# ictnlp/StreamSpeech

Hardware: NVIDIA H100
Metric: audio-seconds/sec (RTF^-1) Fr-En simul S2ST @chunk=320ms (higher is better)
Workload: dtype f32

## Files before the change

### streamspeech_b200/csrc/engine.h

```cpp
#pragma once
#include <cuda_runtime.h>

#include <map>
#include <tuple>
#include <utility>
#include <string>
#include <vector>

#include "../../include/streamspeech_b200.h"
#include "kernels.h"
#include "kernels_persist.h"
#include "kernels_multistream.h"

namespace ss {

struct HostTensor {
  std::vector<float> data;
  std::vector<int64_t> shape;
  int64_t numel() const {
    int64_t n = 1;
    for (auto s : shape) n *= s;
    return n;
  }
};
// ... 12 lines not shown
struct ConformerLayerW {
  LNorm ffn1_ln, ffn2_ln, attn_ln, conv_ln, final_ln;
  Linear ffn1_w1, ffn1_w2, ffn2_w1, ffn2_w2;
  Linear qkv, attn_out;
  float* pos_u = nullptr;
  float* pos_v = nullptr;
  float* pos_proj = nullptr;
  Linear pw1;
  float* dw_w = nullptr;
  float* bn_scale = nullptr;
  float* bn_shift = nullptr;
  Linear pw2;
};

struct DecLayerW {
  LNorm self_ln, cross_ln, final_ln;
  Linear q, k, v, qkv, out;
  Linear cq, ckv, cout;
  Linear fc1, fc2;
  bool has_cross = false;
};

struct ConvW {
  Linear lin;
  int ksize = 1, cin = 0, cout = 0, dil = 1;
};

struct UpsampleW {
  int u = 1, k = 1, pad = 0, cin = 0, cout = 0;
  std::vector<Linear> phase_w;
  std::vector<int> phase_J, phase_q0;
  float* bias = nullptr;
};

struct Arena {
  char* base = nullptr;
  size_t cap = 0, off = 0;
  float* f32(size_t n) { return (float*)raw(n * 4); }
  void* raw(size_t bytes);
  void reset() { off = 0; }
  bool ensure(size_t bytes);
};

}

struct ss_engine {
  int device = 0;
  ss_config cfg{};
  std::string err;
  bool finalized = false;
  int attn_chunk = 8, conv_chunk = 8;
  int umma_vocoder = 0;
  int umma_linear = 0;
  int unit_grouped = 1;
  int umma_min_rows = 128;
  int umma_min_channels = 16;
  ss::Umma2Cache* umma2_cache = nullptr;
  int vocoder_streams = 1;
  cudaStream_t aux_stream[2] = {nullptr, nullptr};
  cudaEvent_t fork_event = nullptr, join_event[2] = {nullptr, nullptr};
  int vocoder_graph = 0;
  int graph_pdl = 0;
  cudaStream_t capture_stream = nullptr;
  std::map<std::tuple<int, uintptr_t, int, int, int>, std::pair<cudaGraphExec_t, int>> voc_graphs;
  int vocoder_fused = -1;
  std::map<std::pair<int, uintptr_t>, ss::VocFusedParams> voc_fused;
  float* persist_ffn_scratch = nullptr;
  float* cl_blobs = nullptr;
  int cluster_cooperative = 1;
  long long cl_steps = 0;
  int persistent_encoder_cluster = 0;
  int persistent_ffn_fused = 1;
  int fbank_tma = 1;
  int persistent_encoder = 1;
  std::map<std::string, ss::HostTensor> host;
  std::vector<void*> dev_allocs;

  ss::Linear sub_conv[2];
  ss::Linear enc_linear;
  std::vector<ss::ConformerLayerW> enc;
  int Tpos = 0;
  ss::Linear ctc_head[2];
  ss::Linear ctc_pair;
  unsigned* ctc_ticket = nullptr;
  float* mt_emb = nullptr;
  float* mt_pos = nullptr;
  int mt_pos_rows = 0;
  std::vector<ss::DecLayerW> mt;
  ss::LNorm mt_ln;
  std::vector<ss::DecLayerW> t2u;
  ss::LNorm t2u_ln;
  std::vector<ss::DecLayerW> unit;
  ss::LNorm unit_ln;
  float* unit_emb = nullptr;
  float* unit_pos_row = nullptr;
  float* mel_bank = nullptr;
  float* melT = nullptr;
  float* window = nullptr;
  float* cmvn_mean = nullptr;
  float* cmvn_std = nullptr;
  float* resample_h = nullptr;
  int resample_taps = 0, resample_width = 0;
  int* mask_pad_unk = nullptr;
  int* mask_pad_eos = nullptr;
  bool has_vocoder = false;
  float* voc_dict = nullptr;
  ss::ConvW dur_conv1, dur_conv2;
  ss::LNorm dur_ln1, dur_ln2;
  ss::Linear dur_proj;
  ss::ConvW conv_pre;
  std::vector<ss::UpsampleW> ups;
  std::vector<std::vector<std::vector<ss::ConvW>>> rb1, rb2;
  float* conv_post_w = nullptr;
  float conv_post_b = 0.f;
  int conv_post_k = 7, conv_post_c = 0;
  int hop = 1, receptive_field = 0;

  ss::Arena ws;
  float* mt_self_k = nullptr;
  float* mt_self_v = nullptr;
  float* mt_cross_kv = nullptr;
  int mt_cross_cap = 0;
  int mt_cross_final = 0;
  int mt_stable_hint = 0;
  const float* mt_cross_enc = nullptr;
  int mt_inc_self_len = 0;
  int mt_inc_cross_rows = 0;
  int64_t* mt_tok_dev = nullptr;
  int64_t* mt_next_dev = nullptr;
  int64_t* mt_next_pinned = nullptr;
  float* voc_unit_emb = nullptr;
  int* voc_cumsum = nullptr;
  int voc_ucap = 0, voc_U = 0;
  int st_T_final = 0;
  float* st_k = nullptr;
  float* st_v = nullptr;
  float* st_glu = nullptr;
  unsigned long long* persist_ts = nullptr;
  int persistent_profile = 0;
  int persistent_prefetch = 0;
  int persistent_time = 0;
  struct TimedLaunch { cudaEvent_t e0, e1; double bytes; };
  std::vector<TimedLaunch> time_events;
  std::vector<TimedLaunch> mt_time_events;
  ss::PersistLayer* persist_alias = nullptr;
  int persistent_alias = 0;
  unsigned* persist_bar = nullptr;
  unsigned persist_bar_target = 0;
  unsigned* async_err_pinned = nullptr;
  int persistent_barrier = 1;
  ss::MtLayerP* mt_persist_layers = nullptr;
  int persistent_mt = 1;
  int persistent_mt_v2 = 1;
  float* mt_part = nullptr;
  int persistent_mt_prefix = 1;
  ss::PersistLayer* persist_layers = nullptr;
  int* lengths_dev = nullptr;
  int lengths_cap = 0;

  struct StreamPool {
    int n_slots = 0, Tcap = 0, Fcap = 0;
    int64_t audio_cap = 0;
    float *audio = nullptr, *feats = nullptr, *k = nullptr, *v = nullptr, *glu = nullptr, *enc_out = nullptr, *melT = nullptr;
    int64_t* ctc_am = nullptr;
    ss::MsStream *desc_dev = nullptr, *desc_pinned = nullptr, *desc_dev2 = nullptr, *desc_pinned2 = nullptr;
    std::vector<int> T_final, n_feat;
    std::vector<int64_t> n_audio;
  } pool;

  int fail(int code, const std::string& msg) {
    err = msg;
    return code;
  }
};
```

### streamspeech_b200/csrc/engine_run.cu

```cuda
#include <algorithm>
#include <cmath>
#include <cstring>
#include <stdexcept>
#include <tuple>

#include "engine.h"

using namespace ss;

namespace {

inline cudaStream_t S(void* s) { return (cudaStream_t)s; }

int check_launch(ss_engine* h, const char* where) {
  cudaError_t e = cudaGetLastError();
  if (e != cudaSuccess) return h->fail(SS_ERR_CUDA, std::string(where) + ": " + cudaGetErrorString(e));
  return SS_OK;
}

thread_local int g_umma_linear = 0;
thread_local int g_umma_conv = 0;
thread_local int g_umma_min_rows = 128;
thread_local int g_umma_min_channels = 16;
thread_local Umma2Cache* g_umma2_cache = nullptr;
// ... 554 lines not shown
  if (T_final_out) *T_final_out = h->st_T_final;
  return check_launch(h, "ss_encoder_stream_step");
}

int ss_ctc_greedy_rows(ss_engine* h, void* stream, int head, const float* enc_dev, int rows, int row0, int64_t* argmax_dev,
                       int64_t* tokens_dev, int32_t* index_dev, int32_t* count_dev) {
  if (h) route_from(h);
  if (!h || !h->finalized) return h ? h->fail(SS_ERR_STATE, "engine not finalized") : SS_ERR_INVALID;
  if (head < 0 || head > 1 || rows <= 0 || row0 < 0 || row0 > rows) return h->fail(SS_ERR_INVALID, "bad ctc head / rows");
  const Linear& l = h->ctc_head[head];
  cudaStream_t st = S(stream);
  const int nr = rows - row0;
  if (nr > 0) {
    if (!ws_begin(h, (size_t)nr * l.N * sizeof(float) + 4096)) return h->fail(SS_ERR_CUDA, "workspace allocation failed");
    float* logits = h->ws.f32((size_t)nr * l.N);
    linear(enc_dev + (size_t)row0 * h->cfg.enc_dim, h->cfg.enc_dim, nr, l, ep_out(logits, l.N), st);
    argmax_rows(logits, l.N, nr, l.N, h->mask_pad_unk, 2, argmax_dev + row0, nullptr, st);
  }
  ctc_collapse(argmax_dev, rows, 0 , h->cfg.pad, tokens_dev, index_dev, count_dev, st);
  return check_launch(h, "ss_ctc_greedy");
}

int ss_ctc_greedy_pair(ss_engine* h, void* stream, const float* enc_dev, int rows, int row0, int64_t* argmax0_dev, int64_t* argmax1_dev,
                       int64_t* packed_out_dev) {
  if (h) route_from(h);
  if (!h || !h->finalized) return h ? h->fail(SS_ERR_STATE, "engine not finalized") : SS_ERR_INVALID;
  if (rows <= 0 || row0 < 0 || row0 > rows) return h->fail(SS_ERR_INVALID, "bad ctc rows");
  cudaStream_t st = S(stream);
  const int V = h->cfg.src_vocab;
  const int nr = rows - row0;
  const int W = 2 * rows + 2;
  if (h->ctc_pair.N != 2 * V || h->cfg.tgt_vocab != V) {
    for (int hd = 0; hd < 2; ++hd) {
      int64_t* o = packed_out_dev + (size_t)hd * W;
      int rc = ss_ctc_greedy_rows(h, stream, hd, enc_dev, rows, row0, hd ? argmax1_dev : argmax0_dev, o + 1, reinterpret_cast<int32_t*>(o + 1 + rows),
                                  reinterpret_cast<int32_t*>(o));
      if (rc) return rc;
    }
    return SS_OK;
  }
  float* logits = nullptr;
  if (nr > 0) {
    if (!ws_begin(h, (size_t)nr * 2 * V * sizeof(float) + 4096)) return h->fail(SS_ERR_CUDA, "workspace allocation failed");
    logits = h->ws.f32((size_t)nr * 2 * V);
    linear(enc_dev + (size_t)row0 * h->cfg.enc_dim, h->cfg.enc_dim, nr, h->ctc_pair, ep_out(logits, 2 * V), st);
  }
  ctc_argmax_collapse_pair(logits, 2 * V, V, nr, row0, rows, h->mask_pad_unk, 2, 0 , h->cfg.pad, argmax0_dev, argmax1_dev,
                           packed_out_dev, W, h->ctc_ticket, st);
  return check_launch(h, "ss_ctc_greedy_pair");
}

int ss_ctc_greedy(ss_engine* h, void* stream, int head, const float* enc_dev, int rows, int64_t* argmax_dev, int64_t* tokens_dev,
                  int32_t* index_dev, int32_t* count_dev) {
  return ss_ctc_greedy_rows(h, stream, head, enc_dev, rows, 0, argmax_dev, tokens_dev, index_dev, count_dev);
}

int ss_mt_features(ss_engine* h, void* stream, const float* enc_dev, int T, const int64_t* tokens_host, int n, float* feats_out_dev,
                   float* logits_last_dev) {
  if (h) route_from(h);
  if (!h || !h->finalized) return h ? h->fail(SS_ERR_STATE, "engine not finalized") : SS_ERR_INVALID;
  const ss_config& c = h->cfg;
  if (n <= 0 || n > c.max_mt_positions || T <= 0) return h->fail(SS_ERR_INVALID, "bad MT sequence length");
  cudaStream_t st = S(stream);
  int rc = ensure_mt_cross(h, T);
  if (rc) return rc;
  int n_valid = n;
  while (n_valid > 0 && tokens_host[n_valid - 1] == c.pad) --n_valid;
  for (int i = 0; i < n_valid; ++i)
    if (tokens_host[i] == c.pad) return h->fail(SS_ERR_INVALID, "pads are only supported as a tail");
  const int dim = c.mt_dim;
  if (!ws_begin(h, ((size_t)n * (dim * 7 + c.mt_ffn) + 4096) * sizeof(float))) return h->fail(SS_ERR_CUDA, "workspace allocation failed");
  DecScratch s = dec_scratch(h, n, dim, c.mt_ffn);
  float* x = h->ws.f32((size_t)n * dim);
  int* kvlen = nullptr;
  cudaMemcpyAsync(h->mt_tok_dev, tokens_host, n * sizeof(int64_t), cudaMemcpyHostToDevice, st);
  if (n_valid < n) {
    kvlen = (int*)h->ws.raw(sizeof(int));
    cudaMemcpyAsync(kvlen, &n_valid, sizeof(int), cudaMemcpyHostToDevice, st);
  }
  cudaStreamSynchronize(st);
  mt_begin(h, enc_dev, T, st);
  mt_forward(h, 0, n, T, kvlen, feats_out_dev, s, x, st);
  if (logits_last_dev) {
    Linear out;
    out.w = h->mt_emb; out.b = nullptr; out.N = c.tgt_vocab; out.K = dim;
    linear(feats_out_dev + (size_t)(n - 1) * dim, dim, 1, out, ep_out(logits_last_dev, c.tgt_vocab), st);
  }
  return check_launch(h, "ss_mt_features");
}

int ss_mt_greedy(ss_engine* h, void* stream, const float* enc_dev, int T, const int64_t* prefix_host, int n_prefix, int max_new_tokens,
                 int max_len_b, int64_t* tokens_out_host, int max_out, int* n_out, float* feats_out_dev) {
  if (h) route_from(h);
  if (!h || !h->finalized) return h ? h->fail(SS_ERR_STATE, "engine not finalized") : SS_ERR_INVALID;
  const ss_config& c = h->cfg;
  cudaStream_t st = S(stream);
  if (T <= 0 || n_prefix < 0 || !n_out) return h->fail(SS_ERR_INVALID, "bad arguments to ss_mt_greedy");
  const int start = n_prefix;
  int max_len = (max_new_tokens == -1) ? std::min(max_len_b, c.max_mt_positions - 1) : start + max_new_tokens;
  if (max_len < 1) return h->fail(SS_ERR_INVALID, "min_len cannot be larger than max_len");
  if (start > max_len) return h->fail(SS_ERR_INVALID, "prefix longer than max_len");
  if (max_len + 2 > c.max_mt_positions || max_len > max_out) return h->fail(SS_ERR_CAPACITY, "MT hypothesis longer than capacity");
  int rc = ensure_mt_cross(h, T);
  if (rc) return rc;
  const int dim = c.mt_dim;
  const int nmax = std::max(start + 1, 1);
  if (!ws_begin(h, ((size_t)nmax * (dim * 7 + c.mt_ffn) + c.tgt_vocab + 4096) * sizeof(float))) return h->fail(SS_ERR_CUDA, "workspace allocation failed");
  DecScratch s = dec_scratch(h, nmax, dim, c.mt_ffn);
  float* x = h->ws.f32((size_t)nmax * dim);
  float* logits = h->ws.f32(c.tgt_vocab);
  Linear outp;
  outp.w = h->mt_emb; outp.b = nullptr; outp.N = c.tgt_vocab; outp.K = dim;
  std::vector<int64_t> toks(start + 1);
  toks[0] = c.eos;
  for (int i = 0; i < start; ++i) toks[i + 1] = prefix_host[i];
  cudaMemcpyAsync(h->mt_tok_dev, toks.data(), toks.size() * sizeof(int64_t), cudaMemcpyHostToDevice, st);
  cudaStreamSynchronize(st);
  mt_begin(h, enc_dev, T, st);
  int fed = 0;
  int n_tok = start;
  for (int i = 0; i < start; ++i) tokens_out_host[i] = prefix_host[i];
  const int burst = (max_new_tokens >= 0) ? std::max(1, max_new_tokens) : 16;
  const bool persistent_mt = h->persistent_mt && mt_decode_persistent_supported(dim, c.mt_ffn, c.mt_heads, c.tgt_vocab, c.max_mt_positions, T);
  int step = start;
  bool done = false;
  if (persistent_mt && h->persistent_mt_prefix && h->persist_bar && start >= 1 && mt_prefix_persistent_supported(dim, c.mt_ffn, c.mt_heads, start, T)) {
    MtDecodeParams P;
    P.n_layers = c.mt_layers; P.heads = c.mt_heads; P.vocab = c.tgt_vocab; P.pad = c.pad; P.eos = c.eos;
    P.max_pos = c.max_mt_positions; P.cross_cap = h->mt_cross_cap;
    P.emb = h->mt_emb; P.pos = h->mt_pos; P.out_g = h->mt_ln.g; P.out_b = h->mt_ln.b;
    P.self_k = h->mt_self_k; P.self_v = h->mt_self_v; P.cross_kv = h->mt_cross_kv;
    P.tok = h->mt_tok_dev; P.feats = feats_out_dev; P.x = x; P.q = s.q; P.attn = s.attn; P.hid = s.hid; P.logits = logits;
        if (h->persistent_mt_v2 && h->mt_part) { P.part = h->mt_part; P.delta = h->mt_part + (size_t)8 * c.mt_dim; }
        if (h->persistent_profile) P.ts = h->persist_ts;
    if (mt_prefix_persistent(P, h->mt_persist_layers, start, T, h->persist_bar, &h->persist_bar_target, st) == 0)
      fed = start;
    else
      cudaGetLastError();
  }
  while (!done) {
    const int burst_first = step;
    int enq = 0;
    for (; step <= max_len && enq < burst; ++step, ++enq) {
      int n = step + 1 - fed;
      if (n == 1 && persistent_mt && h->persist_bar) {
        const int cnt = std::min(max_len - step + 1, burst - enq);
        MtDecodeParams P;
        P.n_layers = c.mt_layers; P.heads = c.mt_heads; P.vocab = c.tgt_vocab; P.pad = c.pad; P.eos = c.eos;
        P.max_pos = c.max_mt_positions; P.cross_cap = h->mt_cross_cap;
        P.emb = h->mt_emb; P.pos = h->mt_pos; P.out_g = h->mt_ln.g; P.out_b = h->mt_ln.b;
        P.self_k = h->mt_self_k; P.self_v = h->mt_self_v; P.cross_kv = h->mt_cross_kv;
        P.tok = h->mt_tok_dev; P.feats = feats_out_dev; P.x = x; P.q = s.q; P.attn = s.attn; P.hid = s.hid; P.logits = logits;
        if (h->persistent_mt_v2 && h->mt_part) { P.part = h->mt_part; P.delta = h->mt_part + (size_t)8 * c.mt_dim; }
        if (h->persistent_profile) P.ts = h->persist_ts;
        cudaEvent_t ev0 = nullptr, ev1 = nullptr;
        if (h->persistent_time && h->mt_time_events.size() < 4096 && cudaEventCreate(&ev0) == cudaSuccess && cudaEventCreate(&ev1) == cudaSuccess)
          cudaEventRecord(ev0, st);
        else
          ev0 = ev1 = nullptr;
        const int rc_launch = mt_decode_persistent(P, h->mt_persist_layers, step, cnt, max_len, T, h->persist_bar, &h->persist_bar_target, st);
        if (ev0 && ev1) {
          cudaEventRecord(ev1, st);
          h->mt_time_events.push_back({ev0, ev1, -1.0});
        }
        if (rc_launch == 0) {
          fed = step + cnt;
          if (step + cnt - 1 >= max_len) done = true;
          step += cnt;
          enq += cnt;
          break;
        }
        cudaGetLastError();
      }
      mt_forward(h, fed, n, T, nullptr, feats_out_dev + (size_t)fed * dim, s, x, st);
      fed = step + 1;
      if (step >= max_len) {
        done = true;
        ++step;
        break;
      }
      linear(feats_out_dev + (size_t)step * dim, dim, 1, outp, ep_out(logits, c.tgt_vocab), st);
      if (step < 1)
        argmax_rows(logits, c.tgt_vocab, 1, c.tgt_vocab, h->mask_pad_eos, 2, h->mt_tok_dev + step + 1, nullptr, st);
      else
        argmax_rows(logits, c.tgt_vocab, 1, c.tgt_vocab, h->mask_pad_unk, 1, h->mt_tok_dev + step + 1, nullptr, st);
    }
    int produced = step - burst_first - (done ? 1 : 0);
    if (produced > 0) {
      cudaMemcpyAsync(h->mt_next_pinned, h->mt_tok_dev + burst_first + 1, produced * sizeof(int64_t), cudaMemcpyDeviceToHost, st);
      if (h->persist_bar && h->async_err_pinned)
        cudaMemcpyAsync(h->async_err_pinned, h->persist_bar + SS_BAR_ERR_WORD, sizeof(unsigned), cudaMemcpyDeviceToHost, st);
      if (cudaStreamSynchronize(st) != cudaSuccess)
        return h->fail(SS_ERR_CUDA, std::string("ss_mt_greedy: ") + cudaGetErrorString(cudaGetLastError()));
      if (h->async_err_pinned && *h->async_err_pinned) {
        const unsigned f = *h->async_err_pinned;
        *h->async_err_pinned = 0;
        return report_async_error(h, f, "ss_mt_greedy");
      }
      int steps_run = produced;
      for (int i = 0; i < produced; ++i) {
        int64_t next = h->mt_next_pinned[i];
        if (next == c.eos) {
          done = true;
          steps_run = i + 1;
          break;
        }
        tokens_out_host[n_tok++] = next;
      }
      if (!h->mt_time_events.empty() && h->mt_time_events.back().bytes < 0.0) h->mt_time_events.back().bytes = (double)steps_run;
    }
    if (step > max_len) done = true;
  }
  *n_out = n_tok;
  return check_launch(h, "ss_mt_greedy");
}

int ss_mt_incremental_reset(ss_engine* h) {
  if (!h) return SS_ERR_INVALID;
  h->mt_inc_self_len = 0;
  h->mt_inc_cross_rows = 0;
  return SS_OK;
}

int ss_mt_greedy_incremental(ss_engine* h, void* stream, const float* enc_dev, int T, const int64_t* prefix_host, int n_prefix,
                             int max_new_tokens, int max_len_b, int64_t* tokens_out_host, int max_out, int* n_out) {
  if (h) route_from(h);
  if (!h || !h->finalized) return h ? h->fail(SS_ERR_STATE, "engine not finalized") : SS_ERR_INVALID;
  const ss_config& c = h->cfg;
  cudaStream_t st = S(stream);
  if (T <= 0 || n_prefix < 0 || !n_out) return h->fail(SS_ERR_INVALID, "bad arguments to ss_mt_greedy_incremental");
  const int start = n_prefix;
  const int max_len = (max_new_tokens == -1) ? max_len_b : start + max_new_tokens;
  if (max_len < 1) return h->fail(SS_ERR_INVALID, "min_len cannot be larger than max_len");
  if (start > max_len) return h->fail(SS_ERR_INVALID, "prefix longer than max_len");
  const int kv_off = h->mt_inc_self_len - start;
  if (kv_off < 0) return h->fail(SS_ERR_STATE, "incremental MT state is shorter than the prefix (reset missing, or a prefix that this state did not produce)");
  if (max_len + kv_off + 2 > c.max_mt_positions || max_len > max_out) return h->fail(SS_ERR_CAPACITY, "MT hypothesis longer than capacity");
  if (!h->persistent_mt || !h->persist_bar || !mt_decode_persistent_supported(c.mt_dim, c.mt_ffn, c.mt_heads, c.tgt_vocab, c.max_mt_positions, std::max(T, h->mt_inc_cross_rows)))
    return h->fail(SS_ERR_STATE, "incremental MT decoding runs on the persistent MT kernel, which is off or does not support this shape");
  int rc = ensure_mt_cross(h, std::max(T, h->mt_inc_cross_rows), h->mt_inc_cross_rows);
  if (rc) return rc;
  const int dim = c.mt_dim;
  if (!ws_begin(h, ((size_t)(dim * 8 + c.mt_ffn) + c.tgt_vocab + (size_t)c.max_mt_positions * dim + 4096) * sizeof(float))) return h->fail(SS_ERR_CUDA, "workspace allocation failed");
  DecScratch s = dec_scratch(h, 1, dim, c.mt_ffn);
  float* x = h->ws.f32(dim);
  float* logits = h->ws.f32(c.tgt_vocab);
  float* feats = h->ws.f32((size_t)c.max_mt_positions * dim);
  if (!x || !logits || !feats) return h->fail(SS_ERR_CUDA, "workspace too small");
  if (h->mt_inc_cross_rows == 0) {
    h->mt_cross_final = 0;
    h->mt_cross_enc = nullptr;
  }
  if (T > h->mt_inc_cross_rows) {
    const int from = h->mt_inc_cross_rows;
    for (int l = 0; l < c.mt_layers; ++l) {
      float* cross = h->mt_cross_kv + (size_t)l * h->mt_cross_cap * 2 * dim;
      linear(enc_dev + (size_t)from * c.enc_dim, c.enc_dim, T - from, h->mt[l].ckv, ep_out(cross + (size_t)from * 2 * dim, 2 * dim), st);
    }
    h->mt_inc_cross_rows = T;
  }
  const int Tk = h->mt_inc_cross_rows;
  std::vector<int64_t> toks(start + 1);
  toks[0] = c.eos;
  for (int i = 0; i < start; ++i) toks[i + 1] = prefix_host[i];
  cudaMemcpyAsync(h->mt_tok_dev, toks.data(), toks.size() * sizeof(int64_t), cudaMemcpyHostToDevice, st);
  cudaStreamSynchronize(st);
  int n_tok = start;
  for (int i = 0; i < start; ++i) tokens_out_host[i] = prefix_host[i];
  const int burst = (max_new_tokens >= 0) ? std::max(1, max_new_tokens + 1) : 32;
  int step = start;
  bool done = false;
  while (!done) {
    const int cnt = std::min(max_len - step + 1, burst);
    MtDecodeParams P;
    P.n_layers = c.mt_layers; P.heads = c.mt_heads; P.vocab = c.tgt_vocab; P.pad = c.pad; P.eos = c.eos;
    P.max_pos = c.max_mt_positions; P.cross_cap = h->mt_cross_cap; P.kv_off = kv_off;
    P.emb = h->mt_emb; P.pos = h->mt_pos; P.out_g = h->mt_ln.g; P.out_b = h->mt_ln.b;
    P.self_k = h->mt_self_k; P.self_v = h->mt_self_v; P.cross_kv = h->mt_cross_kv;
    P.tok = h->mt_tok_dev; P.feats = feats; P.x = x; P.q = s.q; P.attn = s.attn; P.hid = s.hid; P.logits = logits;
        if (h->persistent_mt_v2 && h->mt_part) { P.part = h->mt_part; P.delta = h->mt_part + (size_t)8 * c.mt_dim; }
        if (h->persistent_profile) P.ts = h->persist_ts;
    if (mt_decode_persistent(P, h->mt_persist_layers, step, cnt, max_len, Tk, h->persist_bar, &h->persist_bar_target, st) != 0) {
      cudaGetLastError();
      return h->fail(SS_ERR_CUDA, "cooperative launch of the persistent MT kernel was refused");
    }
    const int readable = std::min(cnt, max_len - step);
    if (readable > 0) cudaMemcpyAsync(h->mt_next_pinned, h->mt_tok_dev + step + 1, readable * sizeof(int64_t), cudaMemcpyDeviceToHost, st);
    if (h->async_err_pinned) cudaMemcpyAsync(h->async_err_pinned, h->persist_bar + SS_BAR_ERR_WORD, sizeof(unsigned), cudaMemcpyDeviceToHost, st);
    if (cudaStreamSynchronize(st) != cudaSuccess) return h->fail(SS_ERR_CUDA, std::string("ss_mt_greedy_incremental: ") + cudaGetErrorString(cudaGetLastError()));
    if (h->async_err_pinned && *h->async_err_pinned) {
      const unsigned f = *h->async_err_pinned;
      *h->async_err_pinned = 0;
      return report_async_error(h, f, "ss_mt_greedy_incremental");
    }
    for (int i = 0; i < cnt && !done; ++i) {
      const int sidx = step + i;
      h->mt_inc_self_len = sidx + kv_off + 1;
      if (sidx >= max_len) { done = true; break; }
      const int64_t next = h->mt_next_pinned[i];
      if (next == c.eos) { done = true; break; }
      tokens_out_host[n_tok++] = next;
    }
    step += cnt;
    if (step > max_len) done = true;
  }
  *n_out = n_tok;
  return check_launch(h, "ss_mt_greedy_incremental");
}

int ss_t2u_unit_decode(ss_engine* h, void* stream, const float* mt_feats_dev, int Slen, int n_pad_tail, int mask_eos, int64_t* argmax_dev,
                       int64_t* units_dev, int32_t* count_dev, float* t2u_out_dev, float* logits_dev) {
  if (h) route_from(h);
  if (!h || !h->finalized) return h ? h->fail(SS_ERR_STATE, "engine not finalized") : SS_ERR_INVALID;
  const ss_config& c = h->cfg;
  cudaStream_t st = S(stream);
  if (Slen <= 0 || n_pad_tail < 0 || n_pad_tail >= Slen) return h->fail(SS_ERR_INVALID, "bad T2U sequence length");
  const int dim = c.unit_dim, R = c.ctc_upsample_rate, L = Slen * R;
  size_t need = ((size_t)L * (dim * 8 + c.unit_ffn + c.unit_vocab) + (size_t)Slen * dim * 12 + (size_t)Slen * c.unit_ffn + 8192) * sizeof(float);
  if (!ws_begin(h, need)) return h->fail(SS_ERR_CUDA, "workspace allocation failed");
  DecScratch s1 = dec_scratch(h, Slen, dim, c.unit_ffn);
  float* x = h->ws.f32((size_t)Slen * dim);
  float* t2u = t2u_out_dev ? t2u_out_dev : h->ws.f32((size_t)Slen * dim);
  int* kvlen = nullptr;
  int* kvlen_up = nullptr;
  if (n_pad_tail > 0) {
    int v[2] = {Slen - n_pad_tail, (Slen - n_pad_tail) * R};
    kvlen = (int*)h->ws.raw(2 * sizeof(int));
    kvlen_up = kvlen + 1;
    cudaMemcpyAsync(kvlen, v, sizeof(v), cudaMemcpyHostToDevice, st);
    cudaStreamSynchronize(st);
  }
  copy_f32(mt_feats_dev, x, (int64_t)Slen * dim, st);
  for (int l = 0; l < c.t2u_layers; ++l)
    dec_layer(h->t2u[l], x, Slen, dim, c.unit_ffn, c.unit_heads, c.uni_encoder != 0, 0, kvlen, nullptr, nullptr, 0, nullptr, 0, nullptr, s1, st);
  layer_norm(x, dim, t2u, dim, h->t2u_ln.g, h->t2u_ln.b, Slen, dim, st);
  DecScratch s2 = dec_scratch(h, L, dim, c.unit_ffn);
  float* xu = h->ws.f32((size_t)L * dim);
  float* ckv = h->ws.f32((size_t)Slen * 2 * dim);
  float* logits = logits_dev ? logits_dev : h->ws.f32((size_t)L * c.unit_vocab);
  if (!xu || !ckv || !logits) return h->fail(SS_ERR_CUDA, "workspace too small");
  repeat_rows_add(t2u, Slen, R, dim, h->unit_pos_row, xu, st);
  for (int l = 0; l < c.unit_layers; ++l) {
    linear(t2u, dim, Slen, h->unit[l].ckv, ep_out(ckv, 2 * dim), st);
    const int gR = (l == 0 && h->unit_grouped) ? R : 0;
    dec_layer(h->unit[l], xu, L, dim, c.unit_ffn, c.unit_heads, true, 0, kvlen_up, nullptr, nullptr, 0, ckv, Slen, kvlen, s2, st, gR, kvlen);
  }
  layer_norm(xu, dim, xu, dim, h->unit_ln.g, h->unit_ln.b, L, dim, st);
  Linear outp;
  outp.w = h->unit_emb; outp.b = nullptr; outp.N = c.unit_vocab; outp.K = dim;
  linear(xu, dim, L, outp, ep_out(logits, c.unit_vocab), st);
  argmax_rows(logits, c.unit_vocab, L, c.unit_vocab, h->mask_pad_unk, mask_eos ? 3 : 2, argmax_dev, nullptr, st);
  ctc_collapse(argmax_dev, L, c.unit_vocab - 1, c.pad, units_dev, nullptr, count_dev, st);
  return check_launch(h, "ss_t2u_unit_decode");
}

int ss_unit_position_row(ss_engine* h, const float* row_host) {
  if (!h || !h->finalized || !row_host) return h ? h->fail(SS_ERR_STATE, "engine not finalized / null row") : SS_ERR_INVALID;
  cudaDeviceSynchronize();
  if (cudaMemcpy(h->unit_pos_row, row_host, (size_t)h->cfg.unit_dim * sizeof(float), cudaMemcpyHostToDevice) != cudaSuccess)
    return h->fail(SS_ERR_CUDA, "cudaMemcpy(unit positional row) failed");
  return SS_OK;
}

int ss_vocoder_durations(ss_engine* h, void* stream, const int64_t* codes_dev, int U, int dur_prediction, int64_t* dur_out_dev,
                         int32_t* cumsum_out_dev) {
  if (!h || !h->finalized) return h ? h->fail(SS_ERR_STATE, "engine not finalized") : SS_ERR_INVALID;
  if (!h->has_vocoder) return h->fail(SS_ERR_STATE, "no vocoder weights were loaded");
  if (U <= 0) return h->fail(SS_ERR_INVALID, "empty code sequence");
  const ss_config& c = h->cfg;
  cudaStream_t st = S(stream);
  const int E = c.voc_embedding_dim, Hd = c.voc_dur_hidden;
  if (U > h->voc_ucap) {
    if (h->voc_unit_emb) cudaFree(h->voc_unit_emb);
    if (h->voc_cumsum) cudaFree(h->voc_cumsum);
    h->voc_unit_emb = nullptr;
    h->voc_cumsum = nullptr;
    h->voc_ucap = 0;
    const int cap = std::max(2 * U, 1024);
    if (cudaMalloc((void**)&h->voc_unit_emb, (size_t)cap * E * sizeof(float)) != cudaSuccess ||
        cudaMalloc((void**)&h->voc_cumsum, (size_t)(cap + 1) * sizeof(int)) != cudaSuccess)
      return h->fail(SS_ERR_CUDA, "cudaMalloc(vocoder unit cache) failed");
    h->voc_ucap = cap;
  }
  h->voc_U = U;
  if (!ws_begin(h, ((size_t)U * (2 * Hd + 2) + 4096) * sizeof(float))) return h->fail(SS_ERR_CUDA, "workspace allocation failed");
  gather_rows(codes_dev, U, 0, h->voc_dict, E, h->voc_unit_emb, st);
  float* a = h->ws.f32((size_t)U * Hd);
  float* b = h->ws.f32((size_t)U * Hd);
  float* ld = h->ws.f32(U);
  if (dur_prediction) {
    ConvA c1;
    c1.x = h->voc_unit_emb; c1.B = 1; c1.L_in = U; c1.L_rows = U; c1.C_in = E; c1.ldx = E;
    c1.ksize = h->dur_conv1.ksize; c1.pad_left = (h->dur_conv1.ksize - 1) / 2;
    Epilogue e1 = ep_out(a, Hd, ACT_RELU);
    e1.bias = h->dur_conv1.lin.b;
    gemm_conv(c1, h->dur_conv1.lin.w, Hd, e1, st);
    layer_norm(a, Hd, a, Hd, h->dur_ln1.g, h->dur_ln1.b, U, Hd, st);
    ConvA c2;
    c2.x = a; c2.B = 1; c2.L_in = U; c2.L_rows = U; c2.C_in = Hd; c2.ldx = Hd;
    c2.ksize = h->dur_conv2.ksize; c2.pad_left = 1;
    Epilogue e2 = ep_out(b, Hd, ACT_RELU);
    e2.bias = h->dur_conv2.lin.b;
    gemm_conv(c2, h->dur_conv2.lin.w, Hd, e2, st);
    layer_norm(b, Hd, b, Hd, h->dur_ln2.g, h->dur_ln2.b, U, Hd, st);
    linear(b, Hd, U, h->dur_proj, ep_out(ld, 1), st);
  } else {
    std::vector<float> v(U, 0.6931472f);
    cudaMemcpyAsync(ld, v.data(), U * sizeof(float), cudaMemcpyHostToDevice, st);
    cudaStreamSynchronize(st);
  }
  duration_from_log(ld, U, dur_out_dev, h->voc_cumsum, st);
  if (cumsum_out_dev) cudaMemcpyAsync(cumsum_out_dev, h->voc_cumsum, (U + 1) * sizeof(int), cudaMemcpyDeviceToDevice, st);
  return check_launch(h, "ss_vocoder_durations");
}

int ss_vocoder_generate(ss_engine* h, void* stream, int total_frames, int frame0, int n_frames, int left_context, float* wav_out_dev) {
  if (!h || !h->finalized) return h ? h->fail(SS_ERR_STATE, "engine not finalized") : SS_ERR_INVALID;
  if (!h->has_vocoder || h->voc_U <= 0) return h->fail(SS_ERR_STATE, "ss_vocoder_durations must run first");
  if (n_frames <= 0 || frame0 < 0 || frame0 + n_frames != total_frames) return h->fail(SS_ERR_INVALID, "vocoder frame range must be the tail of the sequence");
  const ss_config& c = h->cfg;
  cudaStream_t st = S(stream);
  route_from(h);
  g_umma_conv = h->umma_vocoder;
  int ctx = left_context < 0 ? h->receptive_field : left_context;
  ctx = std::min(ctx, frame0);
  const int f_lo = frame0 - ctx;
  const int N = n_frames + ctx;
  size_t maxbuf = 0;
  {
    int ch = c.voc_init_channels;
    size_t L = N;
    maxbuf = L * ch;
    for (int i = 0; i < c.voc_n_ups; ++i) {
// ... 68 lines not shown
      a.pre_lrelu = 0.1f;
      Epilogue e = ep_out(bufY, U.cout);
      e.bias = U.bias;
      e.out_L = Lout; e.out_row_stride = U.u; e.out_row_offset = q0 * U.u + phi - U.pad;
      conv_gemm(a, U.phase_w[phi].w, U.cout, e, sp);
    }
    set_splitk_slot(0);
    if (fan_up)
      for (int q = 0; q < 2; ++q) {
        cudaEventRecord(h->join_event[q], h->aux_stream[q]);
        cudaStreamWaitEvent(st, h->join_event[q], 0);
      }
    L = Lout;
    ch = U.cout;
    if (fan_out) {
      cudaEventRecord(h->fork_event, st);
      for (int q = 0; q < 2; ++q) cudaStreamWaitEvent(h->aux_stream[q], h->fork_event, 0);
    }
    for (int j = 0; j < nrb; ++j) {
      cudaStream_t sj = (fan_out && j > 0) ? h->aux_stream[j - 1] : st;
      set_splitk_slot(fan_out ? j : 0);
      const float* cur = bufY;
      float* pingpong[2] = {rbA[j], rbB[j]};
      int nd = c.voc_rb_ndil;
      for (int m = 0; m < nd; ++m) {
        const ConvW& w1 = h->rb1[i][j][m];
        const ConvW& w2 = h->rb2[i][j][m];
        ConvA a1;
        a1.x = cur; a1.B = 1; a1.L_in = L; a1.L_rows = L; a1.C_in = ch; a1.ldx = ch; a1.ksize = w1.ksize; a1.dil = w1.dil;
        a1.pad_left = (w1.ksize * w1.dil - w1.dil) / 2; a1.pre_lrelu = 0.1f;
        Epilogue e1 = ep_out(rbT[j], ch);
        e1.bias = w1.lin.b;
        conv_gemm(a1, w1.lin.w, ch, e1, sj);
        ConvA a2;
        a2.x = rbT[j]; a2.B = 1; a2.L_in = L; a2.L_rows = L; a2.C_in = ch; a2.ldx = ch; a2.ksize = w2.ksize; a2.dil = 1;
        a2.pad_left = (w2.ksize - 1) / 2; a2.pre_lrelu = 0.1f;
        Epilogue e2;
        e2.bias = w2.lin.b;
        e2.ldo = ch;
        e2.residual = cur;
        if (m + 1 < nd) {
          e2.out = pingpong[m & 1];
          e2.res_scale = 1.0f;
        } else {
          e2.out = nrb == 3 ? rbO[j] : bufX;
          e2.alpha = 1.0f / nrb;
          e2.res_scale = 1.0f / nrb;
          e2.accumulate = nrb != 3 && j > 0;
        }
        conv_gemm(a2, w2.lin.w, ch, e2, sj);
        cur = e2.out;
      }
      if (fan_out && j > 0) cudaEventRecord(h->join_event[j - 1], sj);
    }
    set_splitk_slot(0);
    if (fan_out)
      for (int q = 0; q < 2; ++q) cudaStreamWaitEvent(st, h->join_event[q], 0);
    if (nrb == 3) add3_f32(rbO[0], rbO[1], rbO[2], bufX, (int64_t)L * ch, st);
  }
  conv_post_tanh(bufX, L, ch, h->conv_post_w, h->conv_post_b, h->conv_post_k, 0.01f, wav, st);
  };
  bool replayed = false;
  if (h->vocoder_graph) {
    const auto key = std::make_tuple(N, (uintptr_t)h->ws.base, g_umma_conv, g_umma_min_rows * 4096 + g_umma_min_channels, h->vocoder_streams);
    auto it = h->voc_graphs.find(key);
    if (it != h->voc_graphs.end()) {
      if (cudaGraphLaunch(it->second.first, st) == cudaSuccess) {
        g_launches += it->second.second;
        replayed = true;
      } else {
        cudaGetLastError();
      }
    } else {
      generator_body(st);
      replayed = true;
      if (!h->capture_stream) cudaStreamCreateWithFlags(&h->capture_stream, cudaStreamNonBlocking);
      const unsigned long long before = g_launches;
      if (h->capture_stream && cudaStreamBeginCapture(h->capture_stream, cudaStreamCaptureModeRelaxed) == cudaSuccess) {
        g_pdl_off = h->graph_pdl ? 0 : 1;
        generator_body(h->capture_stream);
        g_pdl_off = 0;
        cudaGraph_t graph = nullptr;
        cudaGraphExec_t exec = nullptr;
        if (cudaStreamEndCapture(h->capture_stream, &graph) == cudaSuccess && graph != nullptr &&
            cudaGraphInstantiate(&exec, graph, 0) == cudaSuccess) {
          h->voc_graphs[key] = std::make_pair(exec, (int)(g_launches - before));
        } else {
          cudaGetLastError();
          h->vocoder_graph = 0;
        }
        if (graph) cudaGraphDestroy(graph);
      } else {
        cudaGetLastError();
        h->vocoder_graph = 0;
      }
      g_launches = before;
    }
  }
  if (!replayed) generator_body(st);
  copy_f32(wav + (size_t)ctx * h->hop, wav_out_dev, (int64_t)n_frames * h->hop, st);
  return check_launch(h, "ss_vocoder_generate");
}

int ss_set_option(ss_engine* h, const char* name, int value) {
  if (!h || !name) return SS_ERR_INVALID;
  std::string n(name);
  if (n == "umma_vocoder") h->umma_vocoder = value;
  else if (n == "umma_linear") h->umma_linear = value;
  else if (n == "umma_min_rows") h->umma_min_rows = value;
  else if (n == "umma_min_channels") h->umma_min_channels = value;
  else if (n == "umma2_cache_clear") {
    umma2_cache_clear(h->umma2_cache);
    clear_graphs(h);
  }
  else if (n == "umma2_split_below") { g_umma2_split_below = value; clear_graphs(h); }
  else if (n == "umma2_min_units") { g_umma2_min_units = value; clear_graphs(h); }
  else if (n == "umma2_debug") {
    if (value && !g_umma2_dbg) {
      if (cudaMalloc(&g_umma2_dbg, 16 * sizeof(unsigned long long)) != cudaSuccess) return h->fail(SS_ERR_CUDA, "cudaMalloc failed");
      cudaMemset(g_umma2_dbg, 0, 16 * sizeof(unsigned long long));
    }
    if (!value && g_umma2_dbg) {
      cudaDeviceSynchronize();
      cudaFree(g_umma2_dbg);
      g_umma2_dbg = nullptr;
    }
  }
  else if (n == "prefer_shared") g_prefer_shared = value;
  else if (n == "unit_grouped") h->unit_grouped = value;
  else if (n == "vocoder_graph") h->vocoder_graph = value;
  else if (n == "vocoder_fused") h->vocoder_fused = value;
  else if (n == "graph_pdl") h->graph_pdl = value;
  else if (n == "fbank_tma") h->fbank_tma = value;
  else if (n == "umma2_fused_reduce") g_umma2_fused_reduce = value;
  else if (n == "persistent_encoder") h->persistent_encoder = value;
  else if (n == "persistent_ffn_fused") h->persistent_ffn_fused = value;
  else if (n == "cluster_cooperative") h->cluster_cooperative = value;
  else if (n == "persistent_encoder_cluster") {
    if (value && !h->cl_blobs) {
      if (!h->persist_layers || !h->persist_bar) return h->fail(SS_ERR_STATE, "persistent_encoder_cluster needs a finalized engine");
      const size_t n_f = encoder_layers_cluster_blob_floats(h->cfg.enc_layers);
      if (h->cfg.enc_dim != 256 || h->cfg.enc_ffn != 2048) return h->fail(SS_ERR_INVALID, "persistent_encoder_cluster: encoder must be 256 / 2048");
      if (cudaMalloc(&h->cl_blobs, n_f * sizeof(float)) != cudaSuccess) return h->fail(SS_ERR_CUDA, "cudaMalloc failed");
      h->dev_allocs.push_back(h->cl_blobs);
      encoder_layers_cluster_pack(h->persist_layers, h->cfg.enc_layers, h->cfg.dw_kernel, h->cl_blobs, 0);
      if (cudaDeviceSynchronize() != cudaSuccess) return h->fail(SS_ERR_CUDA, "packing the cluster weight blobs failed");
    }
    h->persistent_encoder_cluster = value;
  }
  else if (n == "vocoder_streams") h->vocoder_streams = value;
  else if (n == "persistent_mt") h->persistent_mt = value;
  else if (n == "persistent_mt_prefix") h->persistent_mt_prefix = value;
  else if (n == "persistent_mt_v2") h->persistent_mt_v2 = value;
  else if (n == "persistent_prefetch") h->persistent_prefetch = value;
  else if (n == "persistent_time") h->persistent_time = value;
  else if (n == "persistent_barrier") {
    if (value && !h->persist_bar) {
      if (cudaMalloc(&h->persist_bar, 256) != cudaSuccess) return h->fail(SS_ERR_CUDA, "cudaMalloc failed");
      h->dev_allocs.push_back(h->persist_bar);
      cudaMemset(h->persist_bar, 0, 256);
      h->persist_bar_target = 0;
    }
    h->persistent_barrier = value;
  }
  else if (n == "persistent_alias") {
    if (value && !h->persist_alias) {
      const int L = h->cfg.enc_layers;
      if (cudaMalloc(&h->persist_alias, L * sizeof(PersistLayer)) != cudaSuccess) return h->fail(SS_ERR_CUDA, "cudaMalloc failed");
      h->dev_allocs.push_back(h->persist_alias);
      for (int i = 0; i < L; ++i) cudaMemcpy(h->persist_alias + i, h->persist_layers, sizeof(PersistLayer), cudaMemcpyDeviceToDevice);
    }
    h->persistent_alias = value;
  }
  else if (n == "persistent_profile") {
    if (value && !h->persist_ts) {
      if (cudaMalloc(&h->persist_ts, 4096 * sizeof(unsigned long long)) != cudaSuccess) return h->fail(SS_ERR_CUDA, "cudaMalloc failed");
      h->dev_allocs.push_back(h->persist_ts);
    }
    h->persistent_profile = value;
  }
  else return h->fail(SS_ERR_INVALID, "unknown option " + n);
  return SS_OK;
}

int ss_debug_copy(ss_engine* h, const char* what, void* host_dst, size_t bytes) {
  if (!h || !what || !host_dst) return SS_ERR_INVALID;
  std::string n(what);
  if (n == "persist_ts") {
    if (!h->persist_ts || bytes > 4096 * sizeof(unsigned long long)) return h->fail(SS_ERR_STATE, "no phase timestamps (set option persistent_profile)");
    if (cudaMemcpy(host_dst, h->persist_ts, bytes, cudaMemcpyDeviceToHost) != cudaSuccess) return h->fail(SS_ERR_CUDA, "cudaMemcpy failed");
    return SS_OK;
  }
  if (n == "umma2_ts") {
    if (!g_umma2_dbg || bytes > 16 * sizeof(unsigned long long)) return h->fail(SS_ERR_STATE, "no stamps (set option umma2_debug)");
    if (cudaMemcpy(host_dst, g_umma2_dbg, bytes, cudaMemcpyDeviceToHost) != cudaSuccess) return h->fail(SS_ERR_CUDA, "cudaMemcpy failed");
    return SS_OK;
  }
  if (n == "cluster_steps") {
    if (bytes < sizeof(long long)) return h->fail(SS_ERR_INVALID, "cluster_steps needs a long long");
    *(long long*)host_dst = h->cl_steps;
    return SS_OK;
  }
  if (n == "mt_time") {
    if (bytes < 3 * sizeof(double)) return h->fail(SS_ERR_INVALID, "mt_time needs 3 doubles");
    cudaDeviceSynchronize();
    double* out = (double*)host_dst;
    out[0] = out[1] = out[2] = 0.0;
    for (auto& e : h->mt_time_events) {
      float ms = 0.f;
      if (e.bytes >= 0.0 && cudaEventElapsedTime(&ms, e.e0, e.e1) == cudaSuccess) {
        out[0] += ms;
        out[1] += 1.0;
        out[2] += e.bytes;
      }
      cudaEventDestroy(e.e0);
      cudaEventDestroy(e.e1);
    }
    cudaGetLastError();
    h->mt_time_events.clear();
    return SS_OK;
  }
  if (n == "persist_time") {
    if (bytes < 3 * sizeof(double)) return h->fail(SS_ERR_INVALID, "persist_time needs 3 doubles");
    cudaDeviceSynchronize();
    double* out = (double*)host_dst;
    out[0] = out[1] = out[2] = 0.0;
    for (auto& e : h->time_events) {
      float ms = 0.f;
      if (cudaEventElapsedTime(&ms, e.e0, e.e1) == cudaSuccess) {
        out[0] += ms;
        out[1] += 1.0;
        out[2] += e.bytes;
      }
      cudaEventDestroy(e.e0);
      cudaEventDestroy(e.e1);
    }
    cudaGetLastError();
    h->time_events.clear();
    return SS_OK;
  }
  return h->fail(SS_ERR_INVALID, "unknown debug buffer " + n);
}

int ss_op_linear_umma(ss_engine* h, void* stream, const float* x_dev, int M, int K, const float* w_dev, const float* bias_dev, int N, int act,
                      int pieces, float* out_dev) {
  if (!h) return SS_ERR_INVALID;
  route_from(h);
  if (pieces != 2 && pieces != 3) return h->fail(SS_ERR_INVALID, "pieces must be 2 (bf16x3) or 3 (bf16x6)");
  ConvA a;
  a.x = x_dev; a.B = 1; a.L_in = M; a.L_rows = M; a.C_in = K; a.ldx = K;
  Epilogue ep = ep_out(out_dev, N, act);
  ep.bias = bias_dev;
  if (!umma2_supported(a, N, ep)) return h->fail(SS_ERR_INVALID, "shape not supported by the wgmma kernel");
  umma2_conv(h->umma2_cache, a, w_dev, N, ep, pieces, S(stream));
  return check_launch(h, "ss_op_linear_umma");
}

int ss_op_conv1d(ss_engine* h, void* stream, const float* x_dev, int L, int C_in, const float* w_dev, const float* bias_dev, int N, int ksize,
                 int dil, int pad_left, float pre_lrelu, int mode, float* out_dev) {
  if (!h) return SS_ERR_INVALID;
  route_from(h);
  ConvA a;
  a.x = x_dev; a.B = 1; a.L_in = L; a.L_rows = L; a.C_in = C_in; a.ldx = C_in; a.ksize = ksize; a.dil = dil; a.pad_left = pad_left;
  a.pre_lrelu = pre_lrelu;
  Epilogue ep = ep_out(out_dev, N);
  ep.bias = bias_dev;
  if (mode >= 12) {
    if (!umma2_supported(a, N, ep)) return h->fail(SS_ERR_INVALID, "shape not supported by the wgmma conv kernel");
    umma2_conv(h->umma2_cache, a, w_dev, N, ep, mode - 10, S(stream));
  } else if (mode >= 2) {
    return h->fail(SS_ERR_INVALID, "modes 2 / 3 (first-generation tensor-core kernel) were removed: use 12 / 13");
  } else {
    gemm_conv(a, w_dev, N, ep, S(stream));
  }
  return check_launch(h, "ss_op_conv1d");
}

int ss_op_linear(ss_engine* h, void* stream, const float* x_dev, int M, int K, const float* w_dev, const float* bias_dev, int N, int act,
                 float* out_dev) {
  if (!h) return SS_ERR_INVALID;
  Linear l;
  l.w = const_cast<float*>(w_dev); l.b = const_cast<float*>(bias_dev); l.N = N; l.K = K;
  linear(x_dev, K, M, l, ep_out(out_dev, N, act), S(stream));
  return check_launch(h, "ss_op_linear");
}

int ss_op_layer_norm(ss_engine* h, void* stream, const float* x_dev, int rows, int C, const float* g_dev, const float* b_dev, float* out_dev) {
  if (!h) return SS_ERR_INVALID;
  layer_norm(x_dev, C, out_dev, C, g_dev, b_dev, rows, C, S(stream));
  return check_launch(h, "ss_op_layer_norm");
}

}

#include "engine_pool.inc"
```

### streamspeech_b200/csrc/engine_weights.cu

```cuda
#include <cstdio>
#include <cstring>
#include <cmath>
#include <stdexcept>

#include "engine.h"

using namespace ss;

namespace ss {

void* Arena::raw(size_t bytes) {
  size_t a = (off + 255) & ~(size_t)255;
  if (a + bytes > cap) return nullptr;
  off = a + bytes;
  return base + a;
}

bool Arena::ensure(size_t bytes) {
  if (bytes <= cap) return true;
  if (base) cudaFree(base);
  base = nullptr;
  cap = 0;
  size_t want = bytes + (bytes >> 2) + (1 << 20);
  if (cudaMalloc((void**)&base, want) != cudaSuccess) return false;
// ... 146 lines not shown
    {
      std::vector<float> t((size_t)257 * 80);
      for (int m = 0; m < 80; ++m)
        for (int k = 0; k < 257; ++k) t[(size_t)k * 80 + m] = mb.data[(size_t)m * 257 + k];
      h->melT = upload(h, t);
    }
    const HostTensor& w = get(h, "__const__.window");
    expect_shape(w, "__const__.window", {400});
    h->window = upload(h, w.data);
    if (h->host.count("__const__.gcmvn_mean")) {
      h->cmvn_mean = upload(h, get(h, "__const__.gcmvn_mean").data);
      h->cmvn_std = upload(h, get(h, "__const__.gcmvn_std").data);
    }
    if (h->host.count("__const__.resample_3to1")) {
      const HostTensor& r = get(h, "__const__.resample_3to1");
      if (r.numel() < 4 || r.numel() > 64 || (r.numel() - 3) % 2 != 0) throw std::runtime_error("bad __const__.resample_3to1");
      h->resample_h = upload(h, r.data);
      h->resample_taps = (int)r.numel();
      h->resample_width = ((int)r.numel() - 3) / 2;
    }
    int m[3] = {c.pad, c.unk, c.eos};
    h->mask_pad_unk = dev_alloc<int>(h, 3);
    cudaMemcpy(h->mask_pad_unk, m, sizeof(m), cudaMemcpyHostToDevice);
    int m2[2] = {c.pad, c.eos};
    h->mask_pad_eos = dev_alloc<int>(h, 2);
    cudaMemcpy(h->mask_pad_eos, m2, sizeof(m2), cudaMemcpyHostToDevice);
  }
  {
    ConvW c0 = make_conv(h, "encoder.subsample.conv_layers.0", c.conv_channels, c.feat_dim, c.conv_kernel, 1, true);
    ConvW c1 = make_conv(h, "encoder.subsample.conv_layers.1", 2 * D, c.conv_channels / 2, c.conv_kernel, 1, true);
    h->sub_conv[0] = c0.lin;
    h->sub_conv[1] = c1.lin;
    h->enc_linear = make_linear(h, "encoder.linear", D, D);
  }
  const HostTensor& pe = get(h, "__const__.enc_pe");
  h->Tpos = c.max_enc_frames;
  expect_shape(pe, "__const__.enc_pe", {2 * (int64_t)h->Tpos - 1, D});
  std::vector<float> pe_flipped(pe.data.size());
  const int P = 2 * h->Tpos - 1;
  for (int k = 0; k < P; ++k) memcpy(&pe_flipped[(size_t)(P - 1 - k) * D], &pe.data[(size_t)k * D], D * sizeof(float));
  float* pe_dev = upload(h, pe_flipped);
  h->enc.resize(c.enc_layers);
  for (int i = 0; i < c.enc_layers; ++i) {
    ConformerLayerW& L = h->enc[i];
    std::string p = "encoder.conformer_layers." + std::to_string(i);
    L.ffn1_ln = make_ln(h, p + ".ffn1.layer_norm", D);
    L.ffn1_w1 = make_linear(h, p + ".ffn1.w_1", c.enc_ffn, D);
    L.ffn1_w2 = make_linear(h, p + ".ffn1.w_2", D, c.enc_ffn);
    L.ffn2_ln = make_ln(h, p + ".ffn2.layer_norm", D);
    L.ffn2_w1 = make_linear(h, p + ".ffn2.w_1", c.enc_ffn, D);
    L.ffn2_w2 = make_linear(h, p + ".ffn2.w_2", D, c.enc_ffn);
    L.attn_ln = make_ln(h, p + ".self_attn_layer_norm", D);
    L.qkv = make_fused(h, {p + ".self_attn.linear_q", p + ".self_attn.linear_k", p + ".self_attn.linear_v"}, D, D);
    L.attn_out = make_linear(h, p + ".self_attn.linear_out", D, D);
    L.pos_u = upload(h, get(h, p + ".self_attn.pos_bias_u").data);
    L.pos_v = upload(h, get(h, p + ".self_attn.pos_bias_v").data);
    Linear lp = make_linear(h, p + ".self_attn.linear_pos", D, D, false);
    L.pos_proj = dev_alloc<float>(h, (size_t)P * D);
    ConvA a;
    a.x = pe_dev; a.B = 1; a.L_in = P; a.L_rows = P; a.C_in = D; a.ldx = D;
    Epilogue ep;
    ep.out = L.pos_proj; ep.ldo = D;
    gemm_conv(a, lp.w, D, ep, 0);
    L.conv_ln = make_ln(h, p + ".conv_module.layer_norm", D);
    ConvW pw1 = make_conv(h, p + ".conv_module.pointwise_conv1", 2 * D, D, 1, 1, true, false);
    L.pw1 = pw1.lin;
    {
      const HostTensor& dw = get(h, p + ".conv_module.depthwise_conv.weight");
      expect_shape(dw, p + ".conv_module.depthwise_conv.weight", {D, 1, c.dw_kernel});
      std::vector<float> t((size_t)c.dw_kernel * D);
      for (int ch = 0; ch < D; ++ch)
        for (int k = 0; k < c.dw_kernel; ++k) t[(size_t)k * D + ch] = dw.data[(size_t)ch * c.dw_kernel + k];
      L.dw_w = upload(h, t);
      const auto& g = get(h, p + ".conv_module.batch_norm.weight").data;
      const auto& b = get(h, p + ".conv_module.batch_norm.bias").data;
      const auto& rm = get(h, p + ".conv_module.batch_norm.running_mean").data;
      const auto& rv = get(h, p + ".conv_module.batch_norm.running_var").data;
      std::vector<float> sc(D), sh(D);
      for (int ch = 0; ch < D; ++ch) {
        float inv = 1.0f / std::sqrt(rv[ch] + 1e-5f);
        sc[ch] = g[ch] * inv;
        sh[ch] = b[ch] - rm[ch] * g[ch] * inv;
      }
      L.bn_scale = upload(h, sc);
      L.bn_shift = upload(h, sh);
    }
    ConvW pw2 = make_conv(h, p + ".conv_module.pointwise_conv2", D, D, 1, 1, false, false);
    L.pw2 = pw2.lin;
    L.final_ln = make_ln(h, p + ".final_layer_norm", D);
  }
  {
    size_t n = (size_t)c.enc_layers * h->Tpos * D;
    h->st_k = dev_alloc<float>(h, n);
    h->st_v = dev_alloc<float>(h, n);
    h->st_glu = dev_alloc<float>(h, n);
    std::vector<PersistLayer> pl(c.enc_layers);
    for (int i = 0; i < c.enc_layers; ++i) {
      const ConformerLayerW& L = h->enc[i];
      PersistLayer& q = pl[i];
      q.ffn1_g = L.ffn1_ln.g; q.ffn1_b = L.ffn1_ln.b; q.ffn1_w1 = L.ffn1_w1.w; q.ffn1_b1 = L.ffn1_w1.b; q.ffn1_w2 = L.ffn1_w2.w; q.ffn1_b2 = L.ffn1_w2.b;
      q.attn_g = L.attn_ln.g; q.attn_b = L.attn_ln.b; q.wqkv = L.qkv.w; q.bqkv = L.qkv.b; q.wo = L.attn_out.w; q.bo = L.attn_out.b;
      q.pos_u = L.pos_u; q.pos_v = L.pos_v; q.pos_proj = L.pos_proj;
      q.conv_g = L.conv_ln.g; q.conv_b = L.conv_ln.b; q.pw1 = L.pw1.w; q.pw1_b = L.pw1.b; q.dw_w = L.dw_w; q.bn_scale = L.bn_scale;
      q.bn_shift = L.bn_shift; q.pw2 = L.pw2.w; q.pw2_b = L.pw2.b;
      q.ffn2_g = L.ffn2_ln.g; q.ffn2_b = L.ffn2_ln.b; q.ffn2_w1 = L.ffn2_w1.w; q.ffn2_b1 = L.ffn2_w1.b; q.ffn2_w2 = L.ffn2_w2.w; q.ffn2_b2 = L.ffn2_w2.b;
      q.fin_g = L.final_ln.g; q.fin_b = L.final_ln.b;
      for (int which = 0; which < 2; ++which) {
        const HostTensor& w2 = get(h, "encoder.conformer_layers." + std::to_string(&q - pl.data()) + (which ? ".ffn2.w_2.weight" : ".ffn1.w_2.weight"));
        std::vector<float> t((size_t)c.enc_ffn * D);
        for (int n = 0; n < D; ++n)
          for (int u = 0; u < c.enc_ffn; ++u) t[(size_t)u * D + n] = w2.data[(size_t)n * c.enc_ffn + u];
        (which ? q.ffn2_w2t : q.ffn1_w2t) = upload(h, t);
      }
    }
    h->persist_ffn_scratch = dev_alloc<float>(h, (size_t)(c.enc_ffn / 16) * 16 * D);
    h->persist_layers = dev_alloc<PersistLayer>(h, pl.size());
    cudaMemcpy(h->persist_layers, pl.data(), pl.size() * sizeof(PersistLayer), cudaMemcpyHostToDevice);
    h->persist_bar = dev_alloc<unsigned>(h, 64);
    cudaMemset(h->persist_bar, 0, 64 * sizeof(unsigned));
    h->persist_bar_target = 0;
    if (!h->async_err_pinned && cudaHostAlloc((void**)&h->async_err_pinned, sizeof(unsigned), cudaHostAllocDefault) == cudaSuccess)
      *h->async_err_pinned = 0;
  }
  if (c.src_vocab == c.tgt_vocab) {
    h->ctc_pair = make_fused(h, {"source_unigram_decoder.proj", "ctc_target_unigram_decoder.proj"}, c.src_vocab, D);
    h->ctc_head[0] = h->ctc_pair;
    h->ctc_head[0].N = c.src_vocab;
    h->ctc_head[1] = h->ctc_pair;
    h->ctc_head[1].N = c.tgt_vocab;
    h->ctc_head[1].w = h->ctc_pair.w + (size_t)c.src_vocab * D;
    h->ctc_head[1].b = h->ctc_pair.b + c.src_vocab;
  } else {
    h->ctc_head[0] = make_linear(h, "source_unigram_decoder.proj", c.src_vocab, D);
    h->ctc_head[1] = make_linear(h, "ctc_target_unigram_decoder.proj", c.tgt_vocab, D);
  }
  h->ctc_ticket = dev_alloc<unsigned>(h, 8);
  cudaMemset(h->ctc_ticket, 0, 8 * sizeof(unsigned));
  {
    const HostTensor& e = get(h, "target_unigram_decoder.embed_tokens.weight");
    expect_shape(e, "target_unigram_decoder.embed_tokens.weight", {c.tgt_vocab, c.mt_dim});
    h->mt_emb = upload(h, e.data);
    const HostTensor& pt = get(h, "__const__.mt_pos_table");
    if (pt.shape.size() != 2 || pt.shape[1] != c.mt_dim) throw std::runtime_error("bad __const__.mt_pos_table");
    h->mt_pos_rows = (int)pt.shape[0];
    h->mt_pos = upload(h, pt.data);
    for (int i = 0; i < c.mt_layers; ++i)
      h->mt.push_back(make_dec_layer(h, "target_unigram_decoder.layers." + std::to_string(i), c.mt_dim, c.mt_ffn, D, true));
    h->mt_ln = make_ln(h, "target_unigram_decoder.layer_norm", c.mt_dim);
    size_t cache = (size_t)c.mt_layers * c.max_mt_positions * c.mt_dim;
    h->mt_self_k = dev_alloc<float>(h, cache);
    h->mt_self_v = dev_alloc<float>(h, cache);
    h->mt_tok_dev = dev_alloc<int64_t>(h, c.max_mt_positions + 8);
    h->mt_next_dev = dev_alloc<int64_t>(h, 8);
    h->mt_part = dev_alloc<float>(h, (size_t)9 * c.mt_dim);
    cudaMallocHost((void**)&h->mt_next_pinned, (size_t)(c.max_mt_positions + 8) * sizeof(int64_t));
    std::vector<MtLayerP> ml(c.mt_layers);
    for (int i = 0; i < c.mt_layers; ++i) {
      const DecLayerW& L = h->mt[i];
      MtLayerP& q = ml[i];
      q.self_g = L.self_ln.g; q.self_b = L.self_ln.b; q.wqkv = L.qkv.w; q.bqkv = L.qkv.b; q.wo = L.out.w; q.bo = L.out.b;
      q.cross_g = L.cross_ln.g; q.cross_b = L.cross_ln.b; q.wcq = L.cq.w; q.bcq = L.cq.b; q.wco = L.cout.w; q.bco = L.cout.b;
      q.fin_g = L.final_ln.g; q.fin_b = L.final_ln.b; q.w1 = L.fc1.w; q.b1 = L.fc1.b; q.w2 = L.fc2.w; q.b2 = L.fc2.b;
    }
    h->mt_persist_layers = dev_alloc<MtLayerP>(h, ml.size());
    cudaMemcpy(h->mt_persist_layers, ml.data(), ml.size() * sizeof(MtLayerP), cudaMemcpyHostToDevice);
  }
  for (int i = 0; i < c.t2u_layers; ++i)
    h->t2u.push_back(make_dec_layer(h, "synthesizer_encoder.layers." + std::to_string(i), c.unit_dim, c.unit_ffn, c.unit_dim, false));
  h->t2u_ln = make_ln(h, "synthesizer_encoder.layer_norm", c.unit_dim);
  for (int i = 0; i < c.unit_layers; ++i)
    h->unit.push_back(make_dec_layer(h, "decoder.layers." + std::to_string(i), c.unit_dim, c.unit_ffn, c.unit_dim, true));
  h->unit_ln = make_ln(h, "decoder.layer_norm", c.unit_dim);
  {
    const HostTensor& e = get(h, "decoder.embed_tokens.weight");
    expect_shape(e, "decoder.embed_tokens.weight", {c.unit_vocab, c.unit_dim});
    h->unit_emb = upload(h, e.data);
    const HostTensor& pr = get(h, "__const__.unit_pos_row");
    expect_shape(pr, "__const__.unit_pos_row", {c.unit_dim});
    h->unit_pos_row = upload(h, pr.data);
  }
  h->has_vocoder = h->host.count("vocoder.dict.weight") > 0;
  if (h->has_vocoder) {
    const int E = c.voc_embedding_dim;
    const HostTensor& dict = get(h, "vocoder.dict.weight");
    expect_shape(dict, "vocoder.dict.weight", {c.voc_num_embeddings, E});
    h->voc_dict = upload(h, dict.data);
    h->dur_conv1 = make_conv(h, "vocoder.dur_predictor.conv1.0", c.voc_dur_hidden, E, c.voc_dur_kernel, 1, false);
    h->dur_ln1 = make_ln(h, "vocoder.dur_predictor.ln1", c.voc_dur_hidden);
    h->dur_conv2 = make_conv(h, "vocoder.dur_predictor.conv2.0", c.voc_dur_hidden, c.voc_dur_hidden, c.voc_dur_kernel, 1, false);
    h->dur_ln2 = make_ln(h, "vocoder.dur_predictor.ln2", c.voc_dur_hidden);
    h->dur_proj = make_linear(h, "vocoder.dur_predictor.proj", 1, c.voc_dur_hidden);
    h->conv_pre = make_conv(h, "vocoder.conv_pre", c.voc_init_channels, c.voc_in_dim, 7, 1, false);
    int ch = c.voc_init_channels;
    h->hop = 1;
    h->rb1.resize(c.voc_n_ups);
    h->rb2.resize(c.voc_n_ups);
    for (int i = 0; i < c.voc_n_ups; ++i) {
      UpsampleW U;
      U.u = c.voc_up_rates[i];
      U.k = c.voc_up_kernels[i];
      U.pad = (U.k - U.u) / 2;
      U.cin = ch;
      U.cout = ch / 2;
      if ((U.k - U.u) % 2 != 0 || U.pad >= U.u + U.k) throw std::runtime_error("unsupported upsample geometry");
      h->hop *= U.u;
      const std::string p = "vocoder.ups." + std::to_string(i);
      const HostTensor& w = get(h, p + ".weight");
      expect_shape(w, p + ".weight", {U.cin, U.cout, U.k});
      U.bias = upload(h, get(h, p + ".bias").data);
      for (int phi = 0; phi < U.u; ++phi) {
        int J = (U.k - phi + U.u - 1) / U.u;
        std::vector<float> pw((size_t)U.cout * J * U.cin);
        for (int co = 0; co < U.cout; ++co)
          for (int jp = 0; jp < J; ++jp) {
            int kk = phi + (J - 1 - jp) * U.u;
            for (int ci = 0; ci < U.cin; ++ci)
              pw[((size_t)co * J + jp) * U.cin + ci] = w.data[((size_t)ci * U.cout + co) * U.k + kk];
          }
        Linear l;
        l.N = U.cout;
        l.K = J * U.cin;
        l.w = upload(h, pw);
        l.b = U.bias;
        U.phase_w.push_back(l);
        U.phase_J.push_back(J);
        U.phase_q0.push_back(phi < U.pad ? (U.pad - phi + U.u - 1) / U.u : 0);
      }
      h->ups.push_back(U);
      ch = U.cout;
      h->rb1[i].resize(c.voc_n_rb);
      h->rb2[i].resize(c.voc_n_rb);
      for (int j = 0; j < c.voc_n_rb; ++j) {
        int rb = i * c.voc_n_rb + j;
        int rk = c.voc_rb_kernels[j];
        for (int m = 0; m < c.voc_rb_ndil; ++m) {
          std::string q = "vocoder.resblocks." + std::to_string(rb);
          h->rb1[i][j].push_back(make_conv(h, q + ".convs1." + std::to_string(m), ch, ch, rk, c.voc_rb_dils[j][m], false));
          h->rb2[i][j].push_back(make_conv(h, q + ".convs2." + std::to_string(m), ch, ch, rk, 1, false));
        }
      }
    }
    {
      const HostTensor& w = get(h, "vocoder.conv_post.weight");
      expect_shape(w, "vocoder.conv_post.weight", {1, ch, 7});
      std::vector<float> t((size_t)7 * ch);
      for (int ci = 0; ci < ch; ++ci)
        for (int k = 0; k < 7; ++k) t[(size_t)k * ch + ci] = w.data[(size_t)ci * 7 + k];
      h->conv_post_w = upload(h, t);
      h->conv_post_b = get(h, "vocoder.conv_post.bias").data[0];
      h->conv_post_c = ch;
      h->conv_post_k = 7;
    }
    int maxk = 0, sumd = 0;
    for (int j = 0; j < c.voc_n_rb; ++j) {
      int s = 0;
      for (int m = 0; m < c.voc_rb_ndil; ++m) s += c.voc_rb_dils[j][m] + 1;
      int r = (c.voc_rb_kernels[j] - 1) / 2 * s;
      if (r > maxk) maxk = r;
      (void)sumd;
    }
    int r = 3;
    for (int i = c.voc_n_ups - 1; i >= 0; --i) {
      r += maxk;
      r = (r + c.voc_up_kernels[i] + c.voc_up_rates[i] - 1) / c.voc_up_rates[i] + 1;
    }
    h->receptive_field = r + 3;
  }
  if (cudaDeviceSynchronize() != cudaSuccess) throw std::runtime_error(std::string("CUDA error during finalize: ") + cudaGetErrorString(cudaGetLastError()));
  h->host.clear();
  h->finalized = true;
}

}

extern "C" {

const char* ss_version(void) { return "streamspeech_b200 0.1 (sm_90a)"; }

int ss_create(ss_engine** out, int device, const ss_config* cfg) {
  if (!out || !cfg) return SS_ERR_INVALID;
  *out = nullptr;
  int n = 0;
  if (cudaGetDeviceCount(&n) != cudaSuccess || n <= 0 || device >= n) return SS_ERR_CUDA;
  if (cudaSetDevice(device) != cudaSuccess) return SS_ERR_CUDA;
  ss_engine* h = new ss_engine();
  h->device = device;
  h->cfg = *cfg;
  if (h->cfg.voc_n_ups > SS_MAX_UPS || h->cfg.voc_n_rb > SS_MAX_RB || h->cfg.voc_rb_ndil > SS_MAX_DIL) {
    delete h;
    return SS_ERR_INVALID;
  }
  *out = h;
  return SS_OK;
}

int ss_destroy(ss_engine* h) {
  if (!h) return SS_OK;
  cudaSetDevice(h->device);
  cudaDeviceSynchronize();
  for (void* p : h->dev_allocs) cudaFree(p);
  for (auto& kv : h->voc_graphs) cudaGraphExecDestroy(kv.second.first);
  h->voc_graphs.clear();
  if (h->capture_stream) cudaStreamDestroy(h->capture_stream);
  ss::umma2_cache_destroy(h->umma2_cache);
  if (h->ws.base) cudaFree(h->ws.base);
  if (h->mt_cross_kv) cudaFree(h->mt_cross_kv);
  if (h->mt_next_pinned) cudaFreeHost(h->mt_next_pinned);
// ... 58 lines not shown
```

### streamspeech_b200/csrc/kernels_persist.h

```cpp
#pragma once
#include <cuda_runtime.h>
#include <stdint.h>

namespace ss {

#define SS_BAR_ERR_WORD 32

#ifdef __CUDACC__
__device__ __forceinline__ void grid_barrier(unsigned* ctr, unsigned& target) {
  __syncthreads();
  target += gridDim.x;
  if (threadIdx.x == 0) {
    asm volatile("red.release.gpu.global.add.u32 [%0], 1;" ::"l"(ctr) : "memory");
    unsigned v, spins = 0;
    do {
      asm volatile("ld.relaxed.gpu.global.u32 %0, [%1];" : "=r"(v) : "l"(ctr) : "memory");
    } while ((int)(v - target) < 0 && ++spins < (1u << 20));
    if ((int)(v - target) < 0) atomicExch(ctr + SS_BAR_ERR_WORD, 1u);
    asm volatile("fence.acq_rel.gpu;" ::: "memory");
  }
  __syncthreads();
}
#endif

struct PersistLayer {
  const float *ffn1_g, *ffn1_b, *ffn1_w1, *ffn1_b1, *ffn1_w2, *ffn1_b2;
  const float *attn_g, *attn_b, *wqkv, *bqkv, *wo, *bo, *pos_u, *pos_v, *pos_proj;
  const float *conv_g, *conv_b, *pw1, *pw1_b, *dw_w, *bn_scale, *bn_shift, *pw2, *pw2_b;
  const float *ffn2_g, *ffn2_b, *ffn2_w1, *ffn2_b1, *ffn2_w2, *ffn2_b2;
  const float *fin_g, *fin_b;
  const float *ffn1_w2t, *ffn2_w2t;
};

bool encoder_layers_persistent_supported(int nA, int D, int FFN, int H, int T, int dw_k);
int encoder_layers_persistent(const PersistLayer* layers_dev, int n_layers, float* x, float* hid, float* qb, float* att, float* dw, float* kc,
                              float* vc, float* gc, int nA, int a0, int T, int D, int FFN, int H, int Tpos, int chunk, int conv_chunk, int dw_k,
                              unsigned long long* timestamps_or_null, unsigned* barrier_counter_dev_or_null,
                              unsigned* barrier_target_host, int prefetch ,
                              float* ffn_scratch_or_null , cudaStream_t st);

size_t encoder_layers_cluster_blob_floats(int n_layers);
void encoder_layers_cluster_pack(const PersistLayer* layers_dev, int n_layers, int dw_k, float* blobs_dev, cudaStream_t st);
bool encoder_layers_cluster_supported(int nA, int D, int FFN, int H, int T, int dw_k);
int encoder_layers_cluster(const PersistLayer* layers_dev, const float* blobs_dev, int n_layers, float* x, float* kc, float* vc, float* gc, int nA,
                           int a0, int T, int Tpos, int chunk, int conv_chunk, int dw_k, unsigned* bar_ctr, unsigned* bar_target_host,
                           unsigned long long* ts_or_null, const float* const* pos_proj_host , int cooperative ,
                           cudaStream_t st);

struct MtLayerP {
  const float *self_g, *self_b, *wqkv, *bqkv, *wo, *bo;
  const float *cross_g, *cross_b, *wcq, *bcq, *wco, *bco;
  const float *fin_g, *fin_b, *w1, *b1, *w2, *b2;
};
struct MtDecodeParams {
  int n_layers, heads, vocab, pad, eos, max_pos, cross_cap;
  int kv_off = 0;
  const float *emb, *pos, *out_g, *out_b;
  float *self_k, *self_v;
  const float* cross_kv;
  int64_t* tok;
  float* feats;
  float *x, *q, *attn, *hid, *logits;
  unsigned long long* ts = nullptr;
  float *part = nullptr, *delta = nullptr;
};
bool mt_decode_persistent_supported(int dim, int ffn, int heads, int vocab, int max_pos, int T);
int mt_decode_persistent(const MtDecodeParams& P, const MtLayerP* layers_dev, int step0, int nsteps, int max_len, int T,
                         unsigned* barrier_counter_dev, unsigned* barrier_target_host, cudaStream_t st);

bool mt_prefix_persistent_supported(int dim, int ffn, int heads, int M, int T);
int mt_prefix_persistent(const MtDecodeParams& P, const MtLayerP* layers_dev, int M, int T, unsigned* barrier_counter_dev,
                         unsigned* barrier_target_host, cudaStream_t st);

}
```

### streamspeech_b200/csrc/kernels_persist_cl.cu

```cuda
#include <cooperative_groups.h>

#include "common.cuh"
#include "kernels.h"
#include "kernels_persist.h"

namespace cg = cooperative_groups;

namespace ss {
namespace {

constexpr int CT = 256;
constexpr int CWP = CT / 32;
constexpr int CT_ALL = CT + 32;
constexpr int CS = 16;
constexpr int CR = 4;
constexpr int NCL = 4;
constexpr int CD = 256;
constexpr int CHD = 64;
constexpr int NSLOT = 5;
constexpr int SLOT_FLOATS = 32 * CD;
constexpr int CHUNKS_PER_LAYER = 21;

__host__ __device__ constexpr int chunk_rows(int j) { return (j == 9 || j == 10 || j == 12) ? 16 : 32; }
__host__ __device__ constexpr int chunk_row0(int j) {
  int r = 0;
  for (int i = 0; i < j; ++i) r += chunk_rows(i);
  return r;
}
constexpr int BLOB_ROWS = chunk_row0(CHUNKS_PER_LAYER);
constexpr int PO_FFN1_G = 0, PO_FFN1_B = 256, PO_ATTN_G = 512, PO_ATTN_B = 768, PO_CONV_G = 1024, PO_CONV_B = 1280, PO_FFN2_G = 1536,
              PO_FFN2_B = 1792, PO_FIN_G = 2048, PO_FIN_B = 2304, PO_FFN1_B1 = 2560, PO_FFN2_B1 = 2688, PO_FFN1_B2 = 2816, PO_FFN2_B2 = 2832,
              PO_BQKV = 2848, PO_BO = 2896, PO_PW1B = 2912, PO_PW2B = 2944, PO_BN_S = 2960, PO_BN_H = 2976, PO_POSU = 2992, PO_POSV = 3056,
              PO_DW = 3120, PO_END = PO_DW + 31 * 16;
constexpr int PAR_FLOATS = 15 * CD;
static_assert(PO_END <= PAR_FLOATS, "parameter block");
constexpr size_t BLOB_STRIDE = (size_t)PAR_FLOATS + (size_t)BLOB_ROWS * CD;

__device__ __forceinline__ uint32_t smem_u32(const void* p) { return (uint32_t)__cvta_generic_to_shared(p); }

enum { CH_RED = 0, CH_XS = 1, CH_QS = 2, CH_ATTP = 3, CH_AS = 4, N_CH = 5 };

__device__ __forceinline__ uint32_t mapa_u32(uint32_t local, int rank) {
  uint32_t remote;
  asm volatile("mapa.shared::cluster.u32 %0, %1, %2;" : "=r"(remote) : "r"(local), "r"(rank));
  return remote;
}
__device__ __forceinline__ void st_peer(const float* local, int rank, float v, const unsigned long long* bar_local) {
  asm volatile("st.async.weak.shared::cluster.mbarrier::complete_tx::bytes.b32 [%0], %1, [%2];" ::"r"(mapa_u32(smem_u32(local), rank)),
               "r"(__float_as_uint(v)), "r"(mapa_u32(smem_u32(bar_local), rank))
               : "memory");
}

__device__ __forceinline__ void mbar_wait(uint32_t bar, uint32_t parity) {
  uint32_t done = 0;
  while (!done) {
    asm volatile("{\n\t.reg .pred p;\n\tmbarrier.try_wait.parity.shared::cta.b64 p, [%1], %2;\n\tselp.u32 %0, 1, 0, p;\n\t}"
                 : "=r"(done)
                 : "r"(bar), "r"(parity)
                 : "memory");
  }
}

__device__ __forceinline__ unsigned long long globaltimer_ns() {
  unsigned long long t;
  asm volatile("mov.u64 %0, %%globaltimer;" : "=l"(t));
  return t;
}

__device__ __forceinline__ void cluster_sync() {
  asm volatile("barrier.cluster.arrive.release.aligned;\n\tbarrier.cluster.wait.acquire.aligned;" ::: "memory");
}

__device__ __forceinline__ void csync() { asm volatile("bar.sync 1, 256;" ::: "memory"); }

__device__ __forceinline__ void grid_arrive(unsigned* ctr, unsigned& target) {
  csync();
  target += gridDim.x;
  if (threadIdx.x == 0) asm volatile("red.release.gpu.global.add.u32 [%0], 1;" ::"l"(ctr) : "memory");
}
__device__ __forceinline__ void grid_wait(unsigned* ctr, unsigned target) {
  if (threadIdx.x == 0) {
    unsigned v, spins = 0;
    do {
      asm volatile("ld.relaxed.gpu.global.u32 %0, [%1];" : "=r"(v) : "l"(ctr) : "memory");
    } while ((int)(v - target) < 0 && ++spins < (1u << 20));
    if ((int)(v - target) < 0) atomicExch(ctr + SS_BAR_ERR_WORD, 1u);
    asm volatile("fence.acq_rel.gpu;" ::: "memory");
  }
  csync();
}

struct ClSmem {
  float xs[CR][CD];
  float As[CR][CD];
  union {
    struct {
      float hs[CR][128];
      float red[CS][CR][16];
    } f;
    float attp[CS][CR][CHD + 2];
  } u;
  struct {
    float S[CR][256];
    float ml[CR][2];
    float pv[4][CR][CHD];
  } att;
  float qs[CR][CHD];
  float qa[CR][CHD], qb[CR][CHD];
  float outc[CR][48];
  float par[2][PAR_FLOATS];
  unsigned long long full[NSLOT];
  unsigned long long empty[NSLOT];
  unsigned long long parfull[2];
  unsigned long long parfree[2];
  unsigned long long xbar[N_CH];
};

__device__ __noinline__ void stage_ln(ClSmem& sm, const float* g, const float* b) {
  const int lane = threadIdx.x & 31, warp = threadIdx.x >> 5;
  if (warp < CR) {
    float v[8];
#pragma unroll
    for (int i = 0; i < 8; ++i) v[i] = sm.xs[warp][lane + (i << 5)];
    float s = 0.f;
#pragma unroll
    for (int i = 0; i < 8; ++i) s += v[i];
    const float mean = warp_sum(s) / (float)CD;
    float q = 0.f;
#pragma unroll
    for (int i = 0; i < 8; ++i) {
      const float d = v[i] - mean;
      q = fmaf(d, d, q);
    }
    const float rstd = 1.0f / sqrtf(warp_sum(q) / (float)CD + 1e-5f);
#pragma unroll
    for (int i = 0; i < 8; ++i) {
      const int c = lane + (i << 5);
      sm.As[warp][c] = (v[i] - mean) * rstd * g[c] + b[c];
    }
  }
  csync();
}

struct XRegs {
  float4 v[CR][2];
};
__device__ __forceinline__ void load_x(const ClSmem& sm, XRegs& x) {
  const int lane = threadIdx.x & 31;
#pragma unroll
  for (int r = 0; r < CR; ++r) {
    x.v[r][0] = *reinterpret_cast<const float4*>(&sm.As[r][lane * 4]);
    x.v[r][1] = *reinterpret_cast<const float4*>(&sm.As[r][128 + lane * 4]);
  }
}

template <int rows>
__device__ __forceinline__ void chunk_fma(const XRegs& x, const float* wchunk, float (&acc)[16]) {
  const int lane = threadIdx.x & 31, warp = threadIdx.x >> 5;
#pragma unroll
  for (int s = 0; s < 4; ++s) {
    if (s * CWP >= rows) {
#pragma unroll
      for (int r = 0; r < CR; ++r) acc[s * 4 + r] = 0.f;
      continue;
    }
    const float4 w0 = *reinterpret_cast<const float4*>(wchunk + (warp + s * CWP) * CD + lane * 4);
    const float4 w1 = *reinterpret_cast<const float4*>(wchunk + (warp + s * CWP) * CD + 128 + lane * 4);
#pragma unroll
    for (int r = 0; r < CR; ++r) {
      float a = x.v[r][0].x * w0.x;
      a = fmaf(x.v[r][0].y, w0.y, a);
      a = fmaf(x.v[r][0].z, w0.z, a);
      a = fmaf(x.v[r][0].w, w0.w, a);
      a = fmaf(x.v[r][1].x, w1.x, a);
      a = fmaf(x.v[r][1].y, w1.y, a);
      a = fmaf(x.v[r][1].z, w1.z, a);
      a = fmaf(x.v[r][1].w, w1.w, a);
      acc[s * 4 + r] = a;
    }
  }
}

template <int rows>
__device__ __forceinline__ float chunk_tree(const float (&acc)[16]) {
  const int lane = threadIdx.x & 31;
  const bool b4 = lane & 16, b3 = lane & 8, b2 = lane & 4, b1 = lane & 2;
  float w4[4], w2[2];
  if (rows > 16) {
    float w8[8];
#pragma unroll
    for (int i = 0; i < 8; ++i) w8[i] = (b4 ? acc[i + 8] : acc[i]) + __shfl_xor_sync(0xffffffffu, b4 ? acc[i] : acc[i + 8], 16);
#pragma unroll
    for (int i = 0; i < 4; ++i) w4[i] = (b3 ? w8[i + 4] : w8[i]) + __shfl_xor_sync(0xffffffffu, b3 ? w8[i] : w8[i + 4], 8);
  } else {
    float w8[8];
#pragma unroll
    for (int i = 0; i < 8; ++i) w8[i] = acc[i] + __shfl_xor_sync(0xffffffffu, acc[i], 16);
#pragma unroll
    for (int i = 0; i < 4; ++i) w4[i] = (b3 ? w8[i + 4] : w8[i]) + __shfl_xor_sync(0xffffffffu, b3 ? w8[i] : w8[i + 4], 8);
  }
#pragma unroll
  for (int i = 0; i < 2; ++i) w2[i] = (b2 ? w4[i + 2] : w4[i]) + __shfl_xor_sync(0xffffffffu, b2 ? w4[i] : w4[i + 2], 4);
  float v = (b1 ? w2[1] : w2[0]) + __shfl_xor_sync(0xffffffffu, b1 ? w2[0] : w2[1], 2);
  v += __shfl_xor_sync(0xffffffffu, v, 1);
  return v;
}

template <int rows, typename F>
__device__ __forceinline__ void chunk_epi(float v, F&& out) {
  const int lane = threadIdx.x & 31, warp = threadIdx.x >> 5;
  const bool owner = rows > 16 ? (lane & 1) == 0 : (lane & 17) == 0;
  if (owner) {
    const int s = rows > 16 ? (lane >> 3) : ((lane >> 3) & 1);
    out(warp + s * CWP, (lane >> 1) & 3, v);
  }
}

template <int rows, typename F>
__device__ __forceinline__ void chunk_gemm(const XRegs& x, const float* wchunk, F&& out) {
  float acc[16];
  chunk_fma<rows>(x, wchunk, acc);
  chunk_epi<rows>(chunk_tree<rows>(acc), out);
}
// ... 614 lines not shown
```

### streamspeech_b200/csrc/kernels_persist_mt.cu

```cuda
#include "common.cuh"
#include "kernels.h"
#include "kernels_persist.h"

namespace ss {
namespace {

constexpr int MW = 8;
constexpr int MTT = MW * 32;
constexpr int MHD = 64;

__device__ __forceinline__ float4 ldw(const float* p) {
  float4 r;
  asm volatile("ld.global.nc.L1::no_allocate.v4.f32 {%0, %1, %2, %3}, [%4];" : "=f"(r.x), "=f"(r.y), "=f"(r.z), "=f"(r.w) : "l"(p));
  return r;
}

struct MtSmem {
  float x[512];
  float v[2048];
  float S[1024];
  float qh[MHD];
  float pv[16][MHD];
  float red[MW];
  float rbest[MW];
// ... 43 lines not shown
  const int t = threadIdx.x;
  return LnP{__ldg(g + t), __ldg(g + t + MTT), __ldg(b + t), __ldg(b + t + MTT)};
}
__device__ __forceinline__ void ln_to_v(MtSmem& sm, const LnP& p, int dim) {
  const int t = threadIdx.x;
  float a0 = sm.x[t], a1 = sm.x[t + MTT];
  float mean = block_reduce_sum(sm, a0 + a1) / (float)dim;
  float d0 = a0 - mean, d1 = a1 - mean;
  float var = block_reduce_sum(sm, fmaf(d0, d0, d1 * d1)) / (float)dim;
  float rstd = 1.0f / sqrtf(var + 1e-5f);
  sm.v[t] = d0 * rstd * p.g0 + p.b0;
  sm.v[t + MTT] = d1 * rstd * p.g1 + p.b1;
  __syncthreads();
}

__device__ __forceinline__ void load_vec(float* dst, const float* src, int n) {
  for (int i = threadIdx.x * 4; i < n; i += MTT * 4) *reinterpret_cast<float4*>(dst + i) = *reinterpret_cast<const float4*>(src + i);
  __syncthreads();
}

template <int K, int MAXC>
struct GemvW {
  float4 w[MAXC][K / 128];
  float bias[MAXC];
};
template <int K, int MAXC>
__device__ __forceinline__ void gemv_issue(GemvW<K, MAXC>& r, const float* __restrict__ W, int N) {
  const int lane = threadIdx.x & 31;
  const int gw = blockIdx.x * MW + (threadIdx.x >> 5), nw = gridDim.x * MW;
#pragma unroll
  for (int c = 0; c < MAXC; ++c) {
    const int col = gw + c * nw;
#pragma unroll
    for (int it = 0; it < K / 128; ++it)
      r.w[c][it] = col < N ? ldw(W + (int64_t)col * K + it * 128 + lane * 4) : make_float4(0.f, 0.f, 0.f, 0.f);
  }
}
template <int K, int MAXC>
__device__ __forceinline__ void gemv_issue_b(GemvW<K, MAXC>& r, const float* __restrict__ W, int N, const float* __restrict__ bias) {
  gemv_issue(r, W, N);
  const int gw = blockIdx.x * MW + (threadIdx.x >> 5), nw = gridDim.x * MW;
#pragma unroll
  for (int c = 0; c < MAXC; ++c) {
    const int col = gw + c * nw;
    r.bias[c] = (bias != nullptr && col < N) ? __ldg(bias + col) : 0.f;
  }
}
template <int K, int MAXC, typename F>
__device__ __forceinline__ void gemv_finish_b(const GemvW<K, MAXC>& r, const float* xs, int N, F&& epi) {
  constexpr int NIT = K / 128;
  const int lane = threadIdx.x & 31;
  const int gw = blockIdx.x * MW + (threadIdx.x >> 5), nw = gridDim.x * MW;
  float4 xv[NIT];
#pragma unroll
  for (int it = 0; it < NIT; ++it) xv[it] = *reinterpret_cast<const float4*>(xs + it * 128 + lane * 4);
#pragma unroll
  for (int c = 0; c < MAXC; ++c) {
    float acc = 0.f;
#pragma unroll
    for (int it = 0; it < NIT; ++it) {
      acc = fmaf(xv[it].x, r.w[c][it].x, acc);
      acc = fmaf(xv[it].y, r.w[c][it].y, acc);
      acc = fmaf(xv[it].z, r.w[c][it].z, acc);
      acc = fmaf(xv[it].w, r.w[c][it].w, acc);
    }
    acc = warp_sum(acc);
    const int col = gw + c * nw;
    if (lane == 0 && col < N) epi(col, acc + r.bias[c]);
  }
}
template <int K, int MAXC, typename F>
__device__ __forceinline__ void gemv_finish(const GemvW<K, MAXC>& r, const float* xs, int N, F&& epi) {
  constexpr int NIT = K / 128;
  const int lane = threadIdx.x & 31;
  const int gw = blockIdx.x * MW + (threadIdx.x >> 5), nw = gridDim.x * MW;
  float4 xv[NIT];
#pragma unroll
  for (int it = 0; it < NIT; ++it) xv[it] = *reinterpret_cast<const float4*>(xs + it * 128 + lane * 4);
#pragma unroll
  for (int c = 0; c < MAXC; ++c) {
    float acc = 0.f;
#pragma unroll
    for (int it = 0; it < NIT; ++it) {
      acc = fmaf(xv[it].x, r.w[c][it].x, acc);
      acc = fmaf(xv[it].y, r.w[c][it].y, acc);
      acc = fmaf(xv[it].z, r.w[c][it].z, acc);
      acc = fmaf(xv[it].w, r.w[c][it].w, acc);
    }
    acc = warp_sum(acc);
    const int col = gw + c * nw;
    if (lane == 0 && col < N) epi(col, acc);
  }
}

__device__ void attend_head(MtSmem& sm, const float* q, const float* kbase, const float* vbase, int ld, int n, float* out) {
  const int tid = threadIdx.x;
  __syncthreads();
  if (tid < MHD) sm.qh[tid] = q[tid] * 0.125f;
  __syncthreads();
  float mx = -INFINITY;
  for (int j = tid; j < n; j += MTT) {
    const float* kr = kbase + (int64_t)j * ld;
    float4 kk[MHD / 4];
#pragma unroll
    for (int d = 0; d < MHD / 4; ++d) kk[d] = *reinterpret_cast<const float4*>(kr + 4 * d);
    float s = 0.f;
#pragma unroll
    for (int d = 0; d < MHD / 4; ++d) {
      s = fmaf(sm.qh[4 * d], kk[d].x, s);
      s = fmaf(sm.qh[4 * d + 1], kk[d].y, s);
      s = fmaf(sm.qh[4 * d + 2], kk[d].z, s);
      s = fmaf(sm.qh[4 * d + 3], kk[d].w, s);
    }
    sm.S[j] = s;
    mx = fmaxf(mx, s);
  }
  mx = block_reduce_max(sm, mx);
  float sum = 0.f;
  for (int j = tid; j < n; j += MTT) {
    float e = expf(sm.S[j] - mx);
    sm.S[j] = e;
    sum += e;
  }
  sum = block_reduce_sum(sm, sum);
  const int q4 = (tid & 15) * 4, part = tid >> 4;
  float4 a = make_float4(0.f, 0.f, 0.f, 0.f);
#pragma unroll 1
  for (int j0 = part; j0 < n; j0 += 16 * 8) {
    float4 vv[8];
    float pp[8];
#pragma unroll
    for (int u = 0; u < 8; ++u) {
      const int j = j0 + 16 * u;
      const bool ok = j < n;
      vv[u] = ok ? *reinterpret_cast<const float4*>(vbase + (int64_t)j * ld + q4) : make_float4(0.f, 0.f, 0.f, 0.f);
      pp[u] = ok ? sm.S[j] : 0.f;
    }
#pragma unroll
    for (int u = 0; u < 8; ++u) {
      a.x = fmaf(pp[u], vv[u].x, a.x);
      a.y = fmaf(pp[u], vv[u].y, a.y);
      a.z = fmaf(pp[u], vv[u].z, a.z);
      a.w = fmaf(pp[u], vv[u].w, a.w);
    }
  }
  *reinterpret_cast<float4*>(&sm.pv[part][q4]) = a;
  __syncthreads();
  if (tid < MHD) {
    float t = 0.f;
#pragma unroll
    for (int x = 0; x < 16; ++x) t += sm.pv[x][tid];
    out[tid] = t / sum;
  }
}

__global__ void __launch_bounds__(MTT, 1) mt_decode_persistent_kernel(MtDecodeParams P, const MtLayerP* __restrict__ layers, int step0,
                                                                      int nsteps, int max_len, int T, unsigned* bar_ctr,
                                                                      unsigned bar_target) {
  __shared__ __align__(16) MtSmem sm;
  constexpr int DIM = 512, FFN = 2048;
  const int tid = threadIdx.x;
  const int barriers_per_step = P.n_layers * 8 + 1;
  int done_barriers = 0;
  const float emb_scale = sqrtf((float)DIM);
#define BAR()                          \
  grid_barrier(bar_ctr, bar_target);   \
  ++done_barriers;
  for (int si = 0; si < nsteps; ++si) {
    const int s = step0 + si;
    {
      const int64_t tok = (si == 0) ? P.tok[s] : (int64_t)sm.tok;
      const int p = (tok == P.pad) ? P.pad : P.pad + 1 + s;
      for (int c = tid; c < DIM; c += MTT) sm.x[c] = emb_scale * P.emb[tok * DIM + c] + P.pos[(int64_t)p * DIM + c];
      __syncthreads();
    }
    for (int l = 0; l < P.n_layers; ++l) {
      const MtLayerP L = layers[l];
      float* kc = P.self_k + ((size_t)l * P.max_pos + s + P.kv_off) * DIM;
      float* vc = P.self_v + ((size_t)l * P.max_pos + s + P.kv_off) * DIM;
      GemvW<DIM, 2> w_qkv;
      gemv_issue(w_qkv, L.wqkv, 3 * DIM);
      if (l > 0) load_vec(sm.x, P.x, DIM);
      ln_to_v(sm, L.self_g, L.self_b, DIM);
      gemv_finish(w_qkv, sm.v, 3 * DIM, [&](int col, float acc) {
        float y = acc + (L.bqkv ? L.bqkv[col] : 0.f);
        if (col < DIM) P.q[col] = y;
        else if (col < 2 * DIM) kc[col - DIM] = y;
        else vc[col - 2 * DIM] = y;
      });
      BAR();
      if (blockIdx.x < P.heads) {
        const int h = blockIdx.x;
        attend_head(sm, P.q + h * MHD, P.self_k + (size_t)l * P.max_pos * DIM + h * MHD, P.self_v + (size_t)l * P.max_pos * DIM + h * MHD, DIM,
                    s + P.kv_off + 1, P.attn + h * MHD);
      }
      BAR();
      GemvW<DIM, 1> w_o;
      gemv_issue(w_o, L.wo, DIM);
      load_vec(sm.v, P.attn, DIM);
      gemv_finish(w_o, sm.v, DIM, [&](int col, float acc) { P.x[col] = (acc + (L.bo ? L.bo[col] : 0.f)) + sm.x[col]; });
      BAR();
      GemvW<DIM, 1> w_cq;
      gemv_issue(w_cq, L.wcq, DIM);
      load_vec(sm.x, P.x, DIM);
      ln_to_v(sm, L.cross_g, L.cross_b, DIM);
      gemv_finish(w_cq, sm.v, DIM, [&](int col, float acc) { P.q[col] = acc + (L.bcq ? L.bcq[col] : 0.f); });
      BAR();
      if (blockIdx.x < P.heads) {
        const int h = blockIdx.x;
        const float* cross = P.cross_kv + (size_t)l * P.cross_cap * 2 * DIM;
        attend_head(sm, P.q + h * MHD, cross + h * MHD, cross + DIM + h * MHD, 2 * DIM, T, P.attn + h * MHD);
      }
      BAR();
      GemvW<DIM, 1> w_co;
      gemv_issue(w_co, L.wco, DIM);
      load_vec(sm.v, P.attn, DIM);
      gemv_finish(w_co, sm.v, DIM, [&](int col, float acc) { P.x[col] = (acc + (L.bco ? L.bco[col] : 0.f)) + sm.x[col]; });
      BAR();
      GemvW<DIM, 2> w_1;
      gemv_issue(w_1, L.w1, FFN);
      load_vec(sm.x, P.x, DIM);
      ln_to_v(sm, L.fin_g, L.fin_b, DIM);
      gemv_finish(w_1, sm.v, FFN, [&](int col, float acc) {
        float y = acc + (L.b1 ? L.b1[col] : 0.f);
        P.hid[col] = y > 0.f ? y : 0.f;
      });
      BAR();
      GemvW<FFN, 1> w_2;
      gemv_issue(w_2, L.w2, DIM);
      load_vec(sm.v, P.hid, FFN);
      gemv_finish(w_2, sm.v, DIM, [&](int col, float acc) { P.x[col] = (acc + (L.b2 ? L.b2[col] : 0.f)) + sm.x[col]; });
      BAR();
    }
    const bool forced_eos = s >= max_len;
    GemvW<DIM, 6> w_out;
    if (!forced_eos) gemv_issue(w_out, P.emb, P.vocab);
    load_vec(sm.x, P.x, DIM);
    ln_to_v(sm, P.out_g, P.out_b, DIM);
    if (blockIdx.x == 0)
      for (int c = tid; c < DIM; c += MTT) P.feats[(size_t)s * DIM + c] = sm.v[c];
    if (!forced_eos) gemv_finish(w_out, sm.v, P.vocab, [&](int col, float acc) { P.logits[col] = acc; });
    BAR();
    if (forced_eos) break;
    {
      const float* x = P.logits;
      float mx = -INFINITY;
      for (int c = tid; c < P.vocab; c += MTT) mx = fmaxf(mx, x[c]);
      mx = block_reduce_max(sm, mx);
      float su = 0.f;
      for (int c = tid; c < P.vocab; c += MTT) su += expf(x[c] - mx);
      su = block_reduce_sum(sm, su);
      const float lse = logf(su);
      float best = -INFINITY;
      int bi = 0x7fffffff;
      for (int c = tid; c < P.vocab; c += MTT) {
        const bool masked = (c == P.pad) || (s < 1 && c == P.eos);
        float lp = masked ? -INFINITY : (x[c] - mx) - lse;
        if (lp > best || (lp == best && c < bi)) {
          best = lp;
          bi = c;
        }
      }
#pragma unroll
      for (int o = 16; o > 0; o >>= 1) {
        float ob = __shfl_xor_sync(0xffffffffu, best, o);
        int oi = __shfl_xor_sync(0xffffffffu, bi, o);
        if (ob > best || (ob == best && oi < bi)) {
          best = ob;
          bi = oi;
        }
      }
      __syncthreads();
      if ((tid & 31) == 0) {
        sm.rbest[tid >> 5] = best;
        sm.ridx[tid >> 5] = bi;
      }
      __syncthreads();
      if (tid == 0) {
        for (int i = 1; i < MW; ++i)
          if (sm.rbest[i] > best || (sm.rbest[i] == best && sm.ridx[i] < bi)) {
            best = sm.rbest[i];
            bi = sm.ridx[i];
          }
        sm.tok = bi;
        if (blockIdx.x == 0) P.tok[s + 1] = bi;
      }
      __syncthreads();
      if (sm.tok == P.eos) break;
    }
  }
#undef BAR
  const int planned = nsteps * barriers_per_step;
  if (threadIdx.x == 0 && done_barriers < planned) atomicAdd(bar_ctr, (unsigned)(planned - done_barriers));
}

constexpr int GRP = 16;
constexpr int PCOLS = 512 / GRP;
constexpr int PCOLS_PER_WARP = PCOLS / MW;

__device__ void attend_head_early(MtSmem& sm, const float* q, const float* kbase, const float* vbase, int ld, int n, float* out) {
  const int tid = threadIdx.x;
  const int q4 = (tid & 15) * 4, part = tid >> 4;
  float4 kk[MHD / 4];
  {
    const bool ok = tid < n;
    const float* kr = kbase + (int64_t)(ok ? tid : 0) * ld;
#pragma unroll
    for (int d = 0; d < MHD / 4; ++d) kk[d] = ok ? *reinterpret_cast<const float4*>(kr + 4 * d) : make_float4(0.f, 0.f, 0.f, 0.f);
  }
  float4 vv0[8];
#pragma unroll
  for (int u = 0; u < 8; ++u) {
    const int j = part + 16 * u;
    vv0[u] = j < n ? *reinterpret_cast<const float4*>(vbase + (int64_t)j * ld + q4) : make_float4(0.f, 0.f, 0.f, 0.f);
  }
  __syncthreads();
  if (tid < MHD) sm.qh[tid] = q[tid] * 0.125f;
  __syncthreads();
  float mx = -INFINITY;
  for (int j = tid; j < n; j += MTT) {
    if (j != tid) {
      const float* kr = kbase + (int64_t)j * ld;
#pragma unroll
      for (int d = 0; d < MHD / 4; ++d) kk[d] = *reinterpret_cast<const float4*>(kr + 4 * d);
    }
    float s = 0.f;
#pragma unroll
    for (int d = 0; d < MHD / 4; ++d) {
      s = fmaf(sm.qh[4 * d], kk[d].x, s);
      s = fmaf(sm.qh[4 * d + 1], kk[d].y, s);
      s = fmaf(sm.qh[4 * d + 2], kk[d].z, s);
      s = fmaf(sm.qh[4 * d + 3], kk[d].w, s);
    }
    sm.S[j] = s;
    mx = fmaxf(mx, s);
  }
  mx = block_reduce_max(sm, mx);
  float sum = 0.f;
  for (int j = tid; j < n; j += MTT) {
    float e = expf(sm.S[j] - mx);
    sm.S[j] = e;
    sum += e;
  }
  sum = block_reduce_sum(sm, sum);
  float4 a = make_float4(0.f, 0.f, 0.f, 0.f);
#pragma unroll 1
  for (int j0 = part; j0 < n; j0 += 16 * 8) {
    float4 vv[8];
    float pp[8];
#pragma unroll
    for (int u = 0; u < 8; ++u) {
      const int j = j0 + 16 * u;
      const bool ok = j < n;
      vv[u] = j0 == part ? vv0[u] : (ok ? *reinterpret_cast<const float4*>(vbase + (int64_t)j * ld + q4) : make_float4(0.f, 0.f, 0.f, 0.f));
      pp[u] = ok ? sm.S[j] : 0.f;
    }
#pragma unroll
    for (int u = 0; u < 8; ++u) {
      a.x = fmaf(pp[u], vv[u].x, a.x);
      a.y = fmaf(pp[u], vv[u].y, a.y);
      a.z = fmaf(pp[u], vv[u].z, a.z);
      a.w = fmaf(pp[u], vv[u].w, a.w);
    }
  }
  *reinterpret_cast<float4*>(&sm.pv[part][q4]) = a;
  __syncthreads();
  if (tid < MHD) {
    float t = 0.f;
#pragma unroll
    for (int x = 0; x < 16; ++x) t += sm.pv[x][tid];
    out[tid] = t / sum;
  }
}

struct HpW {
  float w0[PCOLS_PER_WARP], w1[PCOLS_PER_WARP];
};

__device__ __forceinline__ HpW hp_load(const float* __restrict__ W, int h, int j) {
  const int lane = threadIdx.x & 31, warp = threadIdx.x >> 5;
  HpW r;
#pragma unroll
  for (int c = 0; c < PCOLS_PER_WARP; ++c) {
    const float* w = W + (int64_t)(j * PCOLS + warp * PCOLS_PER_WARP + c) * 512 + h * MHD;
    r.w0[c] = __ldg(w + lane);
    r.w1[c] = __ldg(w + lane + 32);
  }
  return r;
}
__device__ __forceinline__ void head_partial_proj_w(const float* a, const HpW& hw, int j, float* part_h) {
  const int lane = threadIdx.x & 31, warp = threadIdx.x >> 5;
  const float a0 = a[lane], a1 = a[lane + 32];
#pragma unroll
  for (int c = 0; c < PCOLS_PER_WARP; ++c) {
    float acc = fmaf(a0, hw.w0[c], a1 * hw.w1[c]);
    acc = warp_sum(acc);
    if (lane == 0) part_h[j * PCOLS + warp * PCOLS_PER_WARP + c] = acc;
  }
}

__device__ __forceinline__ void add_head_partials(MtSmem& sm, const float* part, const float* __restrict__ bias) {
  for (int c = threadIdx.x; c < 512; c += MTT) {
    float t = part[c];
#pragma unroll
    for (int h = 1; h < 8; ++h) t += part[h * 512 + c];
    sm.x[c] = sm.x[c] + (t + (bias ? bias[c] : 0.f));
  }
  __syncthreads();
}

template <int K, int MAXC>
__device__ __forceinline__ void gemv_prefetch(const float* __restrict__ W, int N) {
  const int lane = threadIdx.x & 31;
  const int gw = blockIdx.x * MW + (threadIdx.x >> 5), nw = gridDim.x * MW;
  constexpr int LINES = K * 4 / 128;
#pragma unroll
  for (int c = 0; c < MAXC; ++c) {
    const int col = gw + c * nw;
    if (col < N) {
#pragma unroll
      for (int l0 = 0; l0 < LINES; l0 += 32)
        if (l0 + lane < LINES) asm volatile("prefetch.global.L2 [%0];" ::"l"(W + (int64_t)col * K + (l0 + lane) * 32));
    }
  }
}
__device__ __forceinline__ void hp_prefetch(const float* __restrict__ W, int h, int j) {
  const int t = threadIdx.x;
  if (t < PCOLS * 2) asm volatile("prefetch.global.L2 [%0];" ::"l"(W + (int64_t)(j * PCOLS + (t >> 1)) * 512 + h * MHD + (t & 1) * 32));
}
__device__ __forceinline__ void layer_prefetch(const MtLayerP& L, bool in_group, int grp_h, int grp_j) {
  gemv_prefetch<512, 2>(L.wqkv, 3 * 512);
  gemv_prefetch<512, 1>(L.wcq, 512);
  gemv_prefetch<512, 2>(L.w1, 2048);
  gemv_prefetch<2048, 1>(L.w2, 512);
  if (in_group) {
    hp_prefetch(L.wo, grp_h, grp_j);
    hp_prefetch(L.wco, grp_h, grp_j);
  }
}

__device__ __forceinline__ void grid_arrive(unsigned* ctr, unsigned& target) {
  __syncthreads();
  target += gridDim.x;
  if (threadIdx.x == 0) asm volatile("red.release.gpu.global.add.u32 [%0], 1;" ::"l"(ctr) : "memory");
}
__device__ __forceinline__ void grid_wait(unsigned* ctr, unsigned target) {
  if (threadIdx.x == 0) {
    unsigned v, spins = 0;
    do {
      asm volatile("ld.relaxed.gpu.global.u32 %0, [%1];" : "=r"(v) : "l"(ctr) : "memory");
    } while ((int)(v - target) < 0 && ++spins < (1u << 20));
    if ((int)(v - target) < 0) atomicExch(ctr + SS_BAR_ERR_WORD, 1u);
    asm volatile("fence.acq_rel.gpu;" ::: "memory");
  }
  __syncthreads();
}

__global__ void __launch_bounds__(MTT, 1) mt_decode_persistent_kernel_v2(MtDecodeParams P, const MtLayerP* __restrict__ layers, int step0,
                                                                         int nsteps, int max_len, int T, unsigned* bar_ctr,
                                                                         unsigned bar_target) {
  __shared__ __align__(16) MtSmem sm;
  __shared__ __align__(16) float att_h[MHD];
  constexpr int DIM = 512, FFN = 2048;
  const int tid = threadIdx.x;
  const int barriers_per_step = P.n_layers * 6 + 1;
  int done_barriers = 0;
  const float emb_scale = sqrtf((float)DIM);
  const int grp_h = blockIdx.x / GRP, grp_j = blockIdx.x % GRP;
  const bool in_group = blockIdx.x < 8 * GRP;
  float* part = P.part;
  float* delta = P.delta;
#define BAR()                          \
  grid_barrier(bar_ctr, bar_target);   \
  ++done_barriers;
#define ARRIVE()                       \
  grid_arrive(bar_ctr, bar_target);    \
  ++done_barriers;
#define WAIT() grid_wait(bar_ctr, bar_target)
  int nts = 0;
  bool stamping = false;
#define STAMP(id)                                          \
  if (stamping && tid == 0) {                              \
    unsigned long long t_;                                 \
    asm volatile("mov.u64 %0, %%globaltimer;" : "=l"(t_)); \
    P.ts[1 + 2 * nts] = (id);                              \
    P.ts[2 + 2 * nts] = t_;                                \
    ++nts;                                                 \
    P.ts[0] = nts;                                         \
  }
  for (int si = 0; si < nsteps; ++si) {
    const int s = step0 + si;
    {
      const int64_t tok = (si == 0) ? P.tok[s] : (int64_t)sm.tok;
      const int p = (tok == P.pad) ? P.pad : P.pad + 1 + s;
      for (int c = tid; c < DIM; c += MTT) sm.x[c] = emb_scale * P.emb[tok * DIM + c] + P.pos[(int64_t)p * DIM + c];
      __syncthreads();
    }
    GemvW<DIM, 2> w_qkv;
    LnP ln_self;
    {
      const MtLayerP L0 = layers[0];
      gemv_issue_b(w_qkv, L0.wqkv, 3 * DIM, L0.bqkv);
      ln_self = ln_load(L0.self_g, L0.self_b);
    }
    for (int l = 0; l < P.n_layers; ++l) {
      const MtLayerP L = layers[l];
      stamping = P.ts != nullptr && blockIdx.x == 0 && si == 1 && l == 1;
      STAMP(0);
      if (l + 1 < P.n_layers) layer_prefetch(layers[l + 1], in_group, grp_h, grp_j);
      else {
        gemv_prefetch<DIM, 6>(P.emb, P.vocab);
        if (si + 1 < nsteps) layer_prefetch(layers[0], in_group, grp_h, grp_j);
      }
      float* kc = P.self_k + ((size_t)l * P.max_pos + s + P.kv_off) * DIM;
      float* vc = P.self_v + ((size_t)l * P.max_pos + s + P.kv_off) * DIM;
      if (l > 0) {
        for (int c = tid; c < DIM; c += MTT) sm.x[c] = sm.x[c] + delta[c];
        __syncthreads();
      }
      ln_to_v(sm, ln_self, DIM);
      gemv_finish_b(w_qkv, sm.v, 3 * DIM, [&](int col, float y) {
        if (col < DIM) P.q[col] = y;
        else if (col < 2 * DIM) kc[col - DIM] = y;
        else vc[col - 2 * DIM] = y;
      });
      STAMP(1);
      ARRIVE();
      HpW hw;
      if (in_group) hw = hp_load(L.wo, grp_h, grp_j);
      WAIT();
      STAMP(2);
      if (in_group) {
        attend_head_early(sm, P.q + grp_h * MHD, P.self_k + (size_t)l * P.max_pos * DIM + grp_h * MHD, P.self_v + (size_t)l * P.max_pos * DIM + grp_h * MHD,
                          DIM, s + P.kv_off + 1, att_h);
        __syncthreads();
        head_partial_proj_w(att_h, hw, grp_j, part + grp_h * DIM);
      }
      STAMP(3);
      ARRIVE();
      GemvW<DIM, 1> w_cq;
      gemv_issue_b(w_cq, L.wcq, DIM, L.bcq);
      const LnP ln_cross = ln_load(L.cross_g, L.cross_b);
      WAIT();
      STAMP(4);
      add_head_partials(sm, part, L.bo);
      ln_to_v(sm, ln_cross, DIM);
      gemv_finish_b(w_cq, sm.v, DIM, [&](int col, float y) { P.q[col] = y; });
      STAMP(5);
      ARRIVE();
      if (in_group) hw = hp_load(L.wco, grp_h, grp_j);
      WAIT();
      STAMP(6);
      if (in_group) {
        const float* cross = P.cross_kv + (size_t)l * P.cross_cap * 2 * DIM;
        attend_head_early(sm, P.q + grp_h * MHD, cross + grp_h * MHD, cross + DIM + grp_h * MHD, 2 * DIM, T, att_h);
        __syncthreads();
        head_partial_proj_w(att_h, hw, grp_j, part + grp_h * DIM);
      }
      STAMP(7);
      ARRIVE();
      GemvW<DIM, 2> w_1;
      gemv_issue_b(w_1, L.w1, FFN, L.b1);
      const LnP ln_fin = ln_load(L.fin_g, L.fin_b);
      WAIT();
      STAMP(8);
      add_head_partials(sm, part, L.bco);
      ln_to_v(sm, ln_fin, DIM);
      gemv_finish_b(w_1, sm.v, FFN, [&](int col, float y) { P.hid[col] = y > 0.f ? y : 0.f; });
      STAMP(9);
      ARRIVE();
      GemvW<FFN, 1> w_2;
      gemv_issue_b(w_2, L.w2, DIM, L.b2);
      WAIT();
      STAMP(10);
      load_vec(sm.v, P.hid, FFN);
      gemv_finish_b(w_2, sm.v, DIM, [&](int col, float y) { delta[col] = y; });
      STAMP(11);
      ARRIVE();
      if (l + 1 < P.n_layers) {
        const MtLayerP Ln = layers[l + 1];
        gemv_issue_b(w_qkv, Ln.wqkv, 3 * DIM, Ln.bqkv);
        ln_self = ln_load(Ln.self_g, Ln.self_b);
      }
      WAIT();
      STAMP(12);
    }
    const bool forced_eos = s >= max_len;
    GemvW<DIM, 6> w_out;
    if (!forced_eos) gemv_issue(w_out, P.emb, P.vocab);
    const LnP ln_out = ln_load(P.out_g, P.out_b);
    for (int c = tid; c < DIM; c += MTT) sm.x[c] = sm.x[c] + delta[c];
    __syncthreads();
    ln_to_v(sm, ln_out, DIM);
    if (blockIdx.x == 0)
      for (int c = tid; c < DIM; c += MTT) P.feats[(size_t)s * DIM + c] = sm.v[c];
    if (!forced_eos) gemv_finish(w_out, sm.v, P.vocab, [&](int col, float acc) { P.logits[col] = acc; });
    BAR();
    if (forced_eos) break;
    {
      const float* x = P.logits;
      float mx = -INFINITY;
      for (int c = tid; c < P.vocab; c += MTT) mx = fmaxf(mx, x[c]);
      mx = block_reduce_max(sm, mx);
      float su = 0.f;
      for (int c = tid; c < P.vocab; c += MTT) su += expf(x[c] - mx);
      su = block_reduce_sum(sm, su);
      const float lse = logf(su);
      float best = -INFINITY;
      int bi = 0x7fffffff;
      for (int c = tid; c < P.vocab; c += MTT) {
        const bool masked = (c == P.pad) || (s < 1 && c == P.eos);
        float lp = masked ? -INFINITY : (x[c] - mx) - lse;
        if (lp > best || (lp == best && c < bi)) {
          best = lp;
          bi = c;
        }
      }
#pragma unroll
      for (int o = 16; o > 0; o >>= 1) {
        float ob = __shfl_xor_sync(0xffffffffu, best, o);
        int oi = __shfl_xor_sync(0xffffffffu, bi, o);
        if (ob > best || (ob == best && oi < bi)) {
          best = ob;
          bi = oi;
        }
      }
      __syncthreads();
      if ((tid & 31) == 0) {
        sm.rbest[tid >> 5] = best;
        sm.ridx[tid >> 5] = bi;
      }
      __syncthreads();
      if (tid == 0) {
        for (int i = 1; i < MW; ++i)
          if (sm.rbest[i] > best || (sm.rbest[i] == best && sm.ridx[i] < bi)) {
            best = sm.rbest[i];
            bi = sm.ridx[i];
          }
        sm.tok = bi;
        if (blockIdx.x == 0) P.tok[s + 1] = bi;
      }
      __syncthreads();
      if (sm.tok == P.eos) break;
    }
  }
#undef BAR
#undef ARRIVE
#undef WAIT
#undef STAMP
  const int planned = nsteps * barriers_per_step;
  if (threadIdx.x == 0 && done_barriers < planned) atomicAdd(bar_ctr, (unsigned)(planned - done_barriers));
}

}

bool mt_decode_persistent_supported(int dim, int ffn, int heads, int vocab, int max_pos, int T) {
  return vocab <= 6 * MW * 132 && dim == 512 && ffn == 2048 && heads * MHD == dim && vocab >= 1 && max_pos <= 1024 && T >= 1 && T <= 1024;
}

int mt_decode_persistent(const MtDecodeParams& P, const MtLayerP* layers_dev, int step0, int nsteps, int max_len, int T, unsigned* bar_ctr,
                         unsigned* bar_target_host, cudaStream_t st) {
  ++g_launches;
  int occ = 0;
  if (first_time_on_device((const void*)mt_decode_persistent_kernel)) {
    cudaOccupancyMaxActiveBlocksPerMultiprocessor(&occ, mt_decode_persistent_kernel, MTT, 0);
    if (occ < 1) return -1;
  }
  const int grid = current_device_sms();
  if (grid <= 0) return -1;
  if (grid < 128 || P.vocab > 6 * MW * grid) return -1;
  MtDecodeParams p = P;
  unsigned bar_target = *bar_target_host;
  void* args[] = {(void*)&p, (void*)&layers_dev, (void*)&step0, (void*)&nsteps, (void*)&max_len, (void*)&T, (void*)&bar_ctr, (void*)&bar_target};
  const bool v2 = P.part != nullptr && P.delta != nullptr && P.heads == 8 && grid >= 8 * GRP;
  cudaError_t e = cudaLaunchCooperativeKernel(v2 ? (void*)mt_decode_persistent_kernel_v2 : (void*)mt_decode_persistent_kernel, dim3(grid), dim3(MTT), args,
                                              0, st);
  if (e != cudaSuccess) return -2;
  *bar_target_host += (unsigned)grid * (unsigned)(nsteps * (P.n_layers * (v2 ? 6 : 8) + 1));
  return 0;
}

}
```

### streamspeech_b200/engine.py

```python
from __future__ import annotations

import ctypes
import os
from typing import Dict, List, Optional, Sequence, Tuple

import torch

from . import constants
from .config import ModelConfig

_HERE = os.path.dirname(os.path.abspath(__file__))
LIB_PATH = os.path.join(_HERE, "libstreamspeech_b200.so")
SS_MAX_UPS, SS_MAX_RB, SS_MAX_DIL = 8, 4, 4


class SSConfig(ctypes.Structure):
    _fields_ = (
        [(n, ctypes.c_int32) for n in (
            "feat_dim", "enc_dim", "enc_ffn", "enc_heads", "enc_layers", "dw_kernel", "conv_channels", "conv_kernel",
            "src_vocab", "tgt_vocab", "mt_dim", "mt_ffn", "mt_heads", "mt_layers",
            "t2u_layers", "unit_dim", "unit_ffn", "unit_heads", "unit_layers", "unit_vocab", "ctc_upsample_rate",
            "bos", "pad", "eos", "unk", "uni_encoder", "max_enc_frames", "max_mt_positions", "voc_n_ups")]
        + [("voc_up_rates", ctypes.c_int32 * SS_MAX_UPS), ("voc_up_kernels", ctypes.c_int32 * SS_MAX_UPS),
           ("voc_init_channels", ctypes.c_int32), ("voc_n_rb", ctypes.c_int32),
# ... 14 lines not shown
    global _lib
    if _lib is not None:
        return _lib
    if not os.path.exists(LIB_PATH):
        raise EngineError(f"{LIB_PATH} is missing: build it with `make -C streamspeech_b200/csrc` "
                          "(or __graft_entry__.build()).  There is no CPU fallback.")
    lib = ctypes.CDLL(LIB_PATH)
    vp, i32, i64 = ctypes.c_void_p, ctypes.c_int, ctypes.c_int64
    lib.ss_create.argtypes = [ctypes.POINTER(vp), i32, ctypes.POINTER(SSConfig)]
    lib.ss_destroy.argtypes = [vp]
    lib.ss_last_error.argtypes = [vp]
    lib.ss_last_error.restype = ctypes.c_char_p
    lib.ss_version.restype = ctypes.c_char_p
    lib.ss_load_tensor.argtypes = [vp, ctypes.c_char_p, vp, i32, ctypes.POINTER(i64)]
    lib.ss_finalize.argtypes = [vp]
    lib.ss_set_chunk.argtypes = [vp, i32, i32]
    lib.ss_fbank_num_frames.argtypes = [i64]
    lib.ss_fbank_num_frames.restype = i64
    lib.ss_encoder_out_frames.argtypes = [i64]
    lib.ss_encoder_out_frames.restype = i64
    lib.ss_fbank.argtypes = [vp, vp, vp, i64, i64, i64, vp]
    lib.ss_encoder_forward.argtypes = [vp, vp, vp, vp, i32, i32, vp]
    lib.ss_encoder_stream_reset.argtypes = [vp]
    lib.ss_encoder_stream_step.argtypes = [vp, vp, vp, i32, vp, ctypes.POINTER(i32), ctypes.POINTER(i32)]
    lib.ss_ctc_greedy.argtypes = [vp, vp, i32, vp, i32, vp, vp, vp, vp]
    lib.ss_ctc_greedy_rows.argtypes = [vp, vp, i32, vp, i32, i32, vp, vp, vp, vp]
    lib.ss_ctc_greedy_pair.argtypes = [vp, vp, vp, i32, i32, vp, vp, vp]
    lib.ss_mt_greedy.argtypes = [vp, vp, vp, i32, vp, i32, i32, i32, vp, i32, ctypes.POINTER(i32), vp]
    lib.ss_mt_stable_rows.argtypes = [vp, i32]
    lib.ss_mt_incremental_reset.argtypes = [vp]
    lib.ss_mt_greedy_incremental.argtypes = [vp, vp, vp, i32, vp, i32, i32, i32, vp, i32, ctypes.POINTER(i32)]
    lib.ss_mt_features.argtypes = [vp, vp, vp, i32, vp, i32, vp, vp]
    lib.ss_t2u_unit_decode.argtypes = [vp, vp, vp, i32, i32, i32, vp, vp, vp, vp, vp]
    lib.ss_unit_position_row.argtypes = [vp, vp]
    lib.ss_vocoder_durations.argtypes = [vp, vp, vp, i32, i32, vp, vp]
    lib.ss_vocoder_generate.argtypes = [vp, vp, i32, i32, i32, i32, vp]
    lib.ss_vocoder_hop.argtypes = [vp]
    lib.ss_vocoder_receptive_field.argtypes = [vp]
    lib.ss_op_linear.argtypes = [vp, vp, vp, i32, i32, vp, vp, i32, i32, vp]
    lib.ss_op_linear_umma.argtypes = [vp, vp, vp, i32, i32, vp, vp, i32, i32, i32, vp]
    lib.ss_op_conv1d.argtypes = [vp, vp, vp, i32, i32, vp, vp, i32, i32, i32, i32, ctypes.c_float, i32, vp]
    lib.ss_set_option.argtypes = [vp, ctypes.c_char_p, i32]
    lib.ss_op_layer_norm.argtypes = [vp, vp, vp, i32, i32, vp, vp, vp]
    lib.ss_debug_copy.argtypes = [vp, ctypes.c_char_p, vp, ctypes.c_size_t]
    lib.ss_launch_count.argtypes = [vp]
    lib.ss_launch_count.restype = i64
    lib.ss_async_error.argtypes = [vp]
    lib.ss_resample_out_len.argtypes = [i64, i32]
    lib.ss_resample_out_len.restype = i64
    lib.ss_resample_48k_to_16k.argtypes = [vp, vp, vp, i64, i64, i64, vp]
    lib.ss_pool_create.argtypes = [vp, i32, i32]
    lib.ss_pool_reset.argtypes = [vp, i32]
    lib.ss_pool_push_audio.argtypes = [vp, vp, i32, vp, i32]
    lib.ss_pool_info.argtypes = [vp, i32, ctypes.POINTER(i64), ctypes.POINTER(i32), ctypes.POINTER(i32), ctypes.POINTER(vp), ctypes.POINTER(vp)]
    lib.ss_pool_step.argtypes = [vp, vp, i32, vp, i32, vp, i64, vp, vp, vp]
    _lib = lib
    return lib


EXPORTED_SYMBOLS = [
    "ss_create", "ss_destroy", "ss_last_error", "ss_version", "ss_load_tensor", "ss_finalize", "ss_set_chunk",
    "ss_fbank_num_frames", "ss_fbank", "ss_encoder_out_frames", "ss_encoder_forward", "ss_encoder_stream_reset", "ss_encoder_stream_step", "ss_ctc_greedy", "ss_ctc_greedy_rows", "ss_mt_greedy",
    "ss_mt_features", "ss_mt_stable_rows", "ss_t2u_unit_decode", "ss_unit_position_row", "ss_vocoder_durations", "ss_vocoder_generate", "ss_vocoder_hop",
    "ss_vocoder_receptive_field", "ss_op_linear", "ss_op_linear_umma", "ss_op_conv1d", "ss_set_option", "ss_debug_copy", "ss_op_layer_norm", "ss_launch_count", "ss_async_error", "ss_mt_incremental_reset", "ss_mt_greedy_incremental", "ss_ctc_greedy_pair", "ss_resample_out_len", "ss_resample_48k_to_16k", "ss_pool_create", "ss_pool_reset", "ss_pool_push_audio", "ss_pool_info", "ss_pool_step",
]


def make_ss_config(cfg: ModelConfig, max_enc_frames: int, max_mt_positions: int = 1024) -> SSConfig:
    c = SSConfig()
    for n in ("feat_dim", "enc_dim", "enc_ffn", "enc_heads", "enc_layers", "dw_kernel", "conv_channels", "conv_kernel",
              "src_vocab", "tgt_vocab", "mt_dim", "mt_ffn", "mt_heads", "mt_layers", "t2u_layers", "unit_dim", "unit_ffn",
              "unit_heads", "unit_layers", "unit_vocab", "ctc_upsample_rate", "bos", "pad", "eos", "unk"):
        setattr(c, n, int(getattr(cfg, n)))
    c.uni_encoder = int(cfg.uni_encoder)
    c.max_enc_frames = max_enc_frames
    c.max_mt_positions = max_mt_positions
    v = cfg.vocoder
    c.voc_n_ups = len(v.upsample_rates)
    for i, (u, k) in enumerate(zip(v.upsample_rates, v.upsample_kernel_sizes)):
        c.voc_up_rates[i], c.voc_up_kernels[i] = u, k
    c.voc_init_channels = v.upsample_initial_channel
    c.voc_n_rb = len(v.resblock_kernel_sizes)
    c.voc_rb_ndil = len(v.resblock_dilation_sizes[0])
    for j, (k, dils) in enumerate(zip(v.resblock_kernel_sizes, v.resblock_dilation_sizes)):
        c.voc_rb_kernels[j] = k
        assert len(dils) == c.voc_rb_ndil
        for m, d in enumerate(dils):
            c.voc_rb_dils[j][m] = d
    c.voc_num_embeddings, c.voc_embedding_dim, c.voc_in_dim = v.num_embeddings, v.embedding_dim, v.model_in_dim
    c.voc_dur_hidden, c.voc_dur_kernel = v.dur_hidden, v.dur_kernel
    return c


def remove_weight_norm(sd: Dict[str, torch.Tensor]) -> Dict[str, torch.Tensor]:
    out = dict(sd)
    for k in list(sd.keys()):
        if k.endswith(".weight_g"):
            base = k[: -len(".weight_g")]
            g, v = sd[k].float(), sd[base + ".weight_v"].float()
            norm = v.flatten(1).norm(dim=1).view(-1, *([1] * (v.dim() - 1)))
            out[base + ".weight"] = v * (g / norm)
            del out[k], out[base + ".weight_v"]
    return out


class Engine:

    def __init__(self, cfg: ModelConfig, model_sd: Dict[str, torch.Tensor], vocoder_sd: Optional[Dict[str, torch.Tensor]] = None,
                 gcmvn: Optional[dict] = None, device: int = 0, max_enc_frames: int = 1024, max_mt_positions: int = 1024):
        if not torch.cuda.is_available():
            raise EngineError("streamspeech_b200.Engine needs a CUDA device (sm_90a); there is no CPU fallback")
        self.lib = load_library()
        self.cfg = cfg
        self.device = torch.device("cuda", device)
        self.max_mt_positions = max_mt_positions
        self._h = ctypes.c_void_p()
        sc = make_ss_config(cfg, max_enc_frames, max_mt_positions)
        rc = self.lib.ss_create(ctypes.byref(self._h), device, ctypes.byref(sc))
        if rc != 0:
            raise EngineError(f"ss_create failed with {rc}")
        try:
            for k, v in model_sd.items():
                if v.is_floating_point():
                    self._load(k, v)
            if vocoder_sd is not None:
                for k, v in remove_weight_norm(vocoder_sd).items():
                    self._load("vocoder." + k, v)
            self._load("__const__.mel_bank", constants.mel_bank())
            self._load("__const__.window", constants.povey_window())
            self._load("__const__.resample_3to1", constants.resample_kernel_3to1()[0])
            self._load("__const__.enc_pe", constants.rel_pos_table(max_enc_frames, cfg.enc_dim))
            self._load("__const__.mt_pos_table", constants.sinusoidal_table(max_mt_positions + cfg.pad + 2, cfg.mt_dim, cfg.pad))
            self._load("__const__.unit_pos_row", constants.sinusoidal_table(cfg.pad + 4, cfg.unit_dim, cfg.pad)[cfg.pad + 1])
            if gcmvn is not None:
                self._load("__const__.gcmvn_mean", torch.as_tensor(gcmvn["mean"], dtype=torch.float32))
                self._load("__const__.gcmvn_std", torch.as_tensor(gcmvn["std"], dtype=torch.float32))
            self._check(self.lib.ss_finalize(self._h))
        except Exception:
            self.close()
            raise
        self.set_option("prefer_shared", int(os.environ.get("SS_PREFER_SHARED", "0")))
        self.set_option("umma_vocoder", int(os.environ.get("SS_UMMA_VOCODER", "12")))
        self.set_option("umma_linear", int(os.environ.get("SS_UMMA_LINEAR", "13")))
        self.set_option("umma_min_rows", int(os.environ.get("SS_UMMA_MIN_ROWS", "128")))
        self.set_option("umma_min_channels", int(os.environ.get("SS_UMMA_MIN_CHANNELS", "16")))
        self.set_option("persistent_encoder", int(os.environ.get("SS_PERSISTENT_ENCODER", "1")))
        self.set_option("persistent_mt", int(os.environ.get("SS_PERSISTENT_MT", "1")))
        self.set_option("umma2_fused_reduce", int(os.environ.get("SS_UMMA2_FUSED_REDUCE", "0")))
        self.set_option("fbank_tma", int(os.environ.get("SS_FBANK_TMA", "1")))
        self.set_option("persistent_ffn_fused", int(os.environ.get("SS_PERSISTENT_FFN_FUSED", "1")))
        self.set_option("persistent_encoder_cluster", int(os.environ.get("SS_PERSISTENT_ENCODER_CLUSTER", "1")))
        self.set_option("cluster_cooperative", int(os.environ.get("SS_CLUSTER_COOPERATIVE", "1")))
        self.set_option("persistent_mt_v2", int(os.environ.get("SS_PERSISTENT_MT_V2", "1")))
        self.set_option("persistent_mt_prefix", int(os.environ.get("SS_PERSISTENT_MT_PREFIX", "1")))
        self.set_option("vocoder_streams", int(os.environ.get("SS_VOCODER_STREAMS", "1")))
        self.set_option("unit_grouped", int(os.environ.get("SS_UNIT_GROUPED", "1")))
        self.set_option("vocoder_graph", int(os.environ.get("SS_VOCODER_GRAPH", "0")))
        self.set_option("vocoder_fused", int(os.environ.get("SS_VOCODER_FUSED", "-1")))
        self.set_option("graph_pdl", int(os.environ.get("SS_GRAPH_PDL", "0")))
        self.set_option("persistent_prefetch", int(os.environ.get("SS_PERSISTENT_PREFETCH", "0")))
        self.set_option("umma2_split_below", int(os.environ.get("SS_UMMA2_SPLIT_BELOW", "60")))
        self.set_option("umma2_min_units", int(os.environ.get("SS_UMMA2_MIN_UNITS", "4")))
        self.set_option("persistent_barrier", int(os.environ.get("SS_PERSISTENT_BARRIER", "1")))
        self.hop = self.lib.ss_vocoder_hop(self._h)
        self.vocoder_receptive_field = self.lib.ss_vocoder_receptive_field(self._h)

    def close(self):
        if getattr(self, "_h", None) is not None and self._h:
            self.lib.ss_destroy(self._h)
            self._h = None

    def __del__(self):
        try:
            self.close()
        except Exception:
            pass

    def _check(self, rc: int):
        if rc != 0:
            raise EngineError(f"libstreamspeech_b200 error {rc}: {self.lib.ss_last_error(self._h).decode()}")

    def _load(self, key: str, t: torch.Tensor):
        t = t.detach().to(torch.float32).cpu().contiguous()
        shape = (ctypes.c_int64 * max(t.dim(), 1))(*t.shape)
        self._check(self.lib.ss_load_tensor(self._h, key.encode(), t.data_ptr(), t.dim(), shape))

    def _stream(self) -> int:
        return torch.cuda.current_stream(self.device).cuda_stream

    def _f32(self, *shape) -> torch.Tensor:
        return torch.empty(shape, dtype=torch.float32, device=self.device)

    @staticmethod
    def _ptr(t: Optional[torch.Tensor]):
        return None if t is None else t.data_ptr()

    def persistent_phase_stamps(self, n: int):
        buf = (ctypes.c_uint64 * n)()
        self._check(self.lib.ss_debug_copy(self._h, b"persist_ts", ctypes.cast(buf, ctypes.c_void_p), n * 8))
        return list(buf)

    def launch_count(self) -> int:
        return int(self.lib.ss_launch_count(self._h))

    def check_async_error(self):
        self._check(self.lib.ss_async_error(self._h))

    def set_chunk(self, attn_chunk: Optional[int], conv_chunk: Optional[int] = None):
        a = 0 if attn_chunk is None else int(attn_chunk)
        if conv_chunk is None:
            conv_chunk = 0 if attn_chunk is None else (16 if a >= 16 else 8)
        self._check(self.lib.ss_set_chunk(self._h, a, int(conv_chunk)))

    def num_fbank_frames(self, n_samples: int) -> int:
        return int(self.lib.ss_fbank_num_frames(n_samples))

    def encoder_out_frames(self, F: int) -> int:
        return int(self.lib.ss_encoder_out_frames(F))

    def fbank(self, samples: torch.Tensor, frame0: int = 0, n_frames: Optional[int] = None) -> torch.Tensor:
        assert samples.is_cuda and samples.dtype == torch.float32 and samples.is_contiguous()
        F = self.num_fbank_frames(samples.numel())
        if n_frames is None:
            n_frames = F - frame0
        out = self._f32(max(n_frames, 0), self.cfg.feat_dim)
        if n_frames > 0:
            self._check(self.lib.ss_fbank(self._h, self._stream(), samples.data_ptr(), samples.numel(), frame0, n_frames, out.data_ptr()))
        return out

    def resample_out_len(self, n_in_48k: int, finished: bool) -> int:
        return int(self.lib.ss_resample_out_len(int(n_in_48k), int(finished)))

    def resample_48k_to_16k(self, x48: torch.Tensor, out16: torch.Tensor, out0: int, n_out: int):
        assert x48.is_cuda and out16.is_cuda and x48.is_contiguous() and out16.is_contiguous() and out16.numel() >= out0 + n_out
        self._check(self.lib.ss_resample_48k_to_16k(self._h, self._stream(), x48.data_ptr(), x48.numel(), int(out0), int(n_out), out16.data_ptr()))

    def encoder(self, feats: torch.Tensor, lengths: Optional[Sequence[int]] = None) -> torch.Tensor:
        assert feats.is_cuda and feats.dtype == torch.float32 and feats.is_contiguous() and feats.dim() == 3
        B, F, _ = feats.shape
        T = self.encoder_out_frames(F)
        out = self._f32(B, T, self.cfg.enc_dim)
        lens = None
        if lengths is not None:
            lens = (ctypes.c_int32 * B)(*[int(x) for x in lengths])
        self._check(self.lib.ss_encoder_forward(self._h, self._stream(), feats.data_ptr(), lens, B, F, out.data_ptr()))
        return out

    def encoder_stream_reset(self):
        self._check(self.lib.ss_encoder_stream_reset(self._h))

    def encoder_stream_step(self, feats: torch.Tensor, out_buf: torch.Tensor) -> Tuple[int, int]:
        assert feats.is_cuda and feats.is_contiguous() and out_buf.is_cuda and out_buf.is_contiguous()
        T, Tf = ctypes.c_int32(0), ctypes.c_int32(0)
        assert out_buf.shape[0] >= self.encoder_out_frames(feats.shape[0])
        self._check(self.lib.ss_encoder_stream_step(self._h, self._stream(), feats.data_ptr(), feats.shape[0], out_buf.data_ptr(),
                                                    ctypes.byref(T), ctypes.byref(Tf)))
        return T.value, Tf.value

    def ctc_greedy(self, head: int, enc: torch.Tensor):
        assert enc.is_cuda and enc.is_contiguous() and enc.dim() == 2
        T = enc.shape[0]
        am = torch.empty(T, dtype=torch.int64, device=self.device)
        toks = torch.empty(T, dtype=torch.int64, device=self.device)
        idx = torch.empty(T, dtype=torch.int32, device=self.device)
        cnt = torch.zeros(1, dtype=torch.int32, device=self.device)
        self._check(self.lib.ss_ctc_greedy(self._h, self._stream(), head, enc.data_ptr(), T, am.data_ptr(), toks.data_ptr(), idx.data_ptr(), cnt.data_ptr()))
        return {"argmax": am, "tokens": toks, "index": idx, "count": cnt}

    def ctc_greedy_rows(self, head: int, enc: torch.Tensor, row0: int, argmax: torch.Tensor):
        assert enc.is_cuda and enc.is_contiguous() and enc.dim() == 2 and argmax.dtype == torch.int64
        T = enc.shape[0]
        out = torch.empty(2 * T + 2, dtype=torch.int64, device=self.device)
        toks = out[1:1 + T]
        idx = out[1 + T:].view(torch.int32)[:T]
        cnt = out[:1].view(torch.int32)
        cnt.zero_()
        self._check(self.lib.ss_ctc_greedy_rows(self._h, self._stream(), head, enc.data_ptr(), T, int(row0), argmax.data_ptr(), toks.data_ptr(),
                                                idx.data_ptr(), cnt.data_ptr()))
        host = out.cpu()
        n = int(host[:1].view(torch.int32)[0])
        return host[1:1 + n].tolist(), host[1 + T:].view(torch.int32)[:n].tolist()

    def ctc_greedy_rows_pair(self, enc: torch.Tensor, row0s: Sequence[int], argmaxes: Sequence[torch.Tensor]):
        assert enc.is_cuda and enc.is_contiguous() and enc.dim() == 2
        T = enc.shape[0]
        W = 2 * T + 2
        if int(row0s[0]) == int(row0s[1]):
            out = torch.empty(2 * W, dtype=torch.int64, device=self.device)
            self._check(self.lib.ss_ctc_greedy_pair(self._h, self._stream(), enc.data_ptr(), T, int(row0s[0]), argmaxes[0].data_ptr(),
                                                    argmaxes[1].data_ptr(), out.data_ptr()))
        else:
            out = torch.zeros(2 * W, dtype=torch.int64, device=self.device)
            for hd in (0, 1):
                o = out[hd * W:(hd + 1) * W]
                self._check(self.lib.ss_ctc_greedy_rows(self._h, self._stream(), hd, enc.data_ptr(), T, int(row0s[hd]), argmaxes[hd].data_ptr(),
                                                        o[1:1 + T].data_ptr(), o[1 + T:].view(torch.int32)[:T].data_ptr(), o[:1].view(torch.int32).data_ptr()))
        host = out.cpu()
        res = []
        for hd in (0, 1):
            hrow = host[hd * W:(hd + 1) * W]
            n = int(hrow[:1].view(torch.int32)[0])
            res.append((hrow[1:1 + n].tolist(), hrow[1 + T:].view(torch.int32)[:n].tolist()))
        return res[0], res[1]

    def mt_greedy(self, enc: torch.Tensor, prefix: Optional[Sequence[int]], max_new_tokens: int, max_len_b: int = 100,
                  stable_rows: int = 0) -> Tuple[List[int], torch.Tensor]:
# ... 159 lines not shown
```

Measured before the change: 133.2.

## Add thread-block-cluster persistent MT decode kernel with DSMEM head exchange

Adds a new persistent MT greedy-decode kernel launched as thread-block clusters. Each cluster owns an attention head, and peers exchange QKV, cross-query and FFN partial sums through distributed shared memory using st.async and mbarriers, instead of going through global memory and grid-wide barriers. It also factors greedy argmax into a helper, vectorises add_head_partials, and enlarges the partial scratch buffer. The new path is on by default and falls back to the old kernel when occupancy or shape checks fail, at the cost of a complex synchronisation scheme.

```diff
diff --git a/streamspeech_b200/csrc/engine.h b/streamspeech_b200/csrc/engine.h
--- a/streamspeech_b200/csrc/engine.h
+++ b/streamspeech_b200/csrc/engine.h
@@ -188,6 +188,7 @@
   ss::MtLayerP* mt_persist_layers = nullptr;
   int persistent_mt = 1;
   int persistent_mt_v2 = 1;
+  int persistent_mt_cluster = 1;
   float* mt_part = nullptr;
   int persistent_mt_prefix = 1;
   ss::PersistLayer* persist_layers = nullptr;
diff --git a/streamspeech_b200/csrc/engine_run.cu b/streamspeech_b200/csrc/engine_run.cu
--- a/streamspeech_b200/csrc/engine_run.cu
+++ b/streamspeech_b200/csrc/engine_run.cu
@@ -730,6 +730,7 @@
         P.self_k = h->mt_self_k; P.self_v = h->mt_self_v; P.cross_kv = h->mt_cross_kv;
         P.tok = h->mt_tok_dev; P.feats = feats_out_dev; P.x = x; P.q = s.q; P.attn = s.attn; P.hid = s.hid; P.logits = logits;
         if (h->persistent_mt_v2 && h->mt_part) { P.part = h->mt_part; P.delta = h->mt_part + (size_t)8 * c.mt_dim; }
+        if (h->persistent_mt_cluster && h->mt_part) P.part_cl = h->mt_part + (size_t)9 * c.mt_dim;
         if (h->persistent_profile) P.ts = h->persist_ts;
         cudaEvent_t ev0 = nullptr, ev1 = nullptr;
         if (h->persistent_time && h->mt_time_events.size() < 4096 && cudaEventCreate(&ev0) == cudaSuccess && cudaEventCreate(&ev1) == cudaSuccess)
@@ -857,6 +858,7 @@
     P.self_k = h->mt_self_k; P.self_v = h->mt_self_v; P.cross_kv = h->mt_cross_kv;
     P.tok = h->mt_tok_dev; P.feats = feats; P.x = x; P.q = s.q; P.attn = s.attn; P.hid = s.hid; P.logits = logits;
         if (h->persistent_mt_v2 && h->mt_part) { P.part = h->mt_part; P.delta = h->mt_part + (size_t)8 * c.mt_dim; }
+        if (h->persistent_mt_cluster && h->mt_part) P.part_cl = h->mt_part + (size_t)9 * c.mt_dim;
         if (h->persistent_profile) P.ts = h->persist_ts;
     if (mt_decode_persistent(P, h->mt_persist_layers, step, cnt, max_len, Tk, h->persist_bar, &h->persist_bar_target, st) != 0) {
       cudaGetLastError();
@@ -1231,6 +1233,7 @@
   else if (n == "persistent_mt") h->persistent_mt = value;
   else if (n == "persistent_mt_prefix") h->persistent_mt_prefix = value;
   else if (n == "persistent_mt_v2") h->persistent_mt_v2 = value;
+  else if (n == "persistent_mt_cluster") h->persistent_mt_cluster = value;
   else if (n == "persistent_prefetch") h->persistent_prefetch = value;
   else if (n == "persistent_time") h->persistent_time = value;
   else if (n == "persistent_barrier") {
diff --git a/streamspeech_b200/csrc/engine_weights.cu b/streamspeech_b200/csrc/engine_weights.cu
--- a/streamspeech_b200/csrc/engine_weights.cu
+++ b/streamspeech_b200/csrc/engine_weights.cu
@@ -322,7 +322,7 @@
     h->mt_self_v = dev_alloc<float>(h, cache);
     h->mt_tok_dev = dev_alloc<int64_t>(h, c.max_mt_positions + 8);
     h->mt_next_dev = dev_alloc<int64_t>(h, 8);
-    h->mt_part = dev_alloc<float>(h, (size_t)9 * c.mt_dim);
+    h->mt_part = dev_alloc<float>(h, (size_t)(9 + 24) * c.mt_dim);
     cudaMallocHost((void**)&h->mt_next_pinned, (size_t)(c.max_mt_positions + 8) * sizeof(int64_t));
     std::vector<MtLayerP> ml(c.mt_layers);
     for (int i = 0; i < c.mt_layers; ++i) {
diff --git a/streamspeech_b200/csrc/kernels_persist.h b/streamspeech_b200/csrc/kernels_persist.h
--- a/streamspeech_b200/csrc/kernels_persist.h
+++ b/streamspeech_b200/csrc/kernels_persist.h
@@ -20,6 +20,33 @@
     asm volatile("fence.acq_rel.gpu;" ::: "memory");
   }
   __syncthreads();
+}
+
+__device__ __forceinline__ uint32_t smem_u32(const void* p) { return (uint32_t)__cvta_generic_to_shared(p); }
+
+__device__ __forceinline__ uint32_t mapa_u32(uint32_t local, int rank) {
+  uint32_t remote;
+  asm volatile("mapa.shared::cluster.u32 %0, %1, %2;" : "=r"(remote) : "r"(local), "r"(rank));
+  return remote;
+}
+__device__ __forceinline__ void st_peer(const float* local, int rank, float v, const unsigned long long* bar_local) {
+  asm volatile("st.async.weak.shared::cluster.mbarrier::complete_tx::bytes.b32 [%0], %1, [%2];" ::"r"(mapa_u32(smem_u32(local), rank)),
+               "r"(__float_as_uint(v)), "r"(mapa_u32(smem_u32(bar_local), rank))
+               : "memory");
+}
+
+__device__ __forceinline__ void mbar_wait(uint32_t bar, uint32_t parity) {
+  uint32_t done = 0;
+  while (!done) {
+    asm volatile("{\n\t.reg .pred p;\n\tmbarrier.try_wait.parity.shared::cta.b64 p, [%1], %2;\n\tselp.u32 %0, 1, 0, p;\n\t}"
+                 : "=r"(done)
+                 : "r"(bar), "r"(parity)
+                 : "memory");
+  }
+}
+
+__device__ __forceinline__ void cluster_sync() {
+  asm volatile("barrier.cluster.arrive.release.aligned;\n\tbarrier.cluster.wait.acquire.aligned;" ::: "memory");
 }
 #endif
 
@@ -63,6 +90,7 @@
   float *x, *q, *attn, *hid, *logits;
   unsigned long long* ts = nullptr;
   float *part = nullptr, *delta = nullptr;
+  float* part_cl = nullptr;
 };
 bool mt_decode_persistent_supported(int dim, int ffn, int heads, int vocab, int max_pos, int T);
 int mt_decode_persistent(const MtDecodeParams& P, const MtLayerP* layers_dev, int step0, int nsteps, int max_len, int T,
diff --git a/streamspeech_b200/csrc/kernels_persist_cl.cu b/streamspeech_b200/csrc/kernels_persist_cl.cu
--- a/streamspeech_b200/csrc/kernels_persist_cl.cu
+++ b/streamspeech_b200/csrc/kernels_persist_cl.cu
@@ -36,39 +36,13 @@
 static_assert(PO_END <= PAR_FLOATS, "parameter block");
 constexpr size_t BLOB_STRIDE = (size_t)PAR_FLOATS + (size_t)BLOB_ROWS * CD;
 
-__device__ __forceinline__ uint32_t smem_u32(const void* p) { return (uint32_t)__cvta_generic_to_shared(p); }
 
 enum { CH_RED = 0, CH_XS = 1, CH_QS = 2, CH_ATTP = 3, CH_AS = 4, N_CH = 5 };
-
-__device__ __forceinline__ uint32_t mapa_u32(uint32_t local, int rank) {
-  uint32_t remote;
-  asm volatile("mapa.shared::cluster.u32 %0, %1, %2;" : "=r"(remote) : "r"(local), "r"(rank));
-  return remote;
-}
-__device__ __forceinline__ void st_peer(const float* local, int rank, float v, const unsigned long long* bar_local) {
-  asm volatile("st.async.weak.shared::cluster.mbarrier::complete_tx::bytes.b32 [%0], %1, [%2];" ::"r"(mapa_u32(smem_u32(local), rank)),
-               "r"(__float_as_uint(v)), "r"(mapa_u32(smem_u32(bar_local), rank))
-               : "memory");
-}
-
-__device__ __forceinline__ void mbar_wait(uint32_t bar, uint32_t parity) {
-  uint32_t done = 0;
-  while (!done) {
-    asm volatile("{\n\t.reg .pred p;\n\tmbarrier.try_wait.parity.shared::cta.b64 p, [%1], %2;\n\tselp.u32 %0, 1, 0, p;\n\t}"
-                 : "=r"(done)
-                 : "r"(bar), "r"(parity)
-                 : "memory");
-  }
-}
 
 __device__ __forceinline__ unsigned long long globaltimer_ns() {
   unsigned long long t;
   asm volatile("mov.u64 %0, %%globaltimer;" : "=l"(t));
   return t;
-}
-
-__device__ __forceinline__ void cluster_sync() {
-  asm volatile("barrier.cluster.arrive.release.aligned;\n\tbarrier.cluster.wait.acquire.aligned;" ::: "memory");
 }
 
 __device__ __forceinline__ void csync() { asm volatile("bar.sync 1, 256;" ::: "memory"); }
diff --git a/streamspeech_b200/csrc/kernels_persist_mt.cu b/streamspeech_b200/csrc/kernels_persist_mt.cu
--- a/streamspeech_b200/csrc/kernels_persist_mt.cu
+++ b/streamspeech_b200/csrc/kernels_persist_mt.cu
@@ -219,6 +219,52 @@
     for (int x = 0; x < 16; ++x) t += sm.pv[x][tid];
     out[tid] = t / sum;
   }
+}
+
+__device__ void greedy_argmax(MtSmem& sm, const MtDecodeParams& P, int s, const float* x) {
+  const int tid = threadIdx.x;
+  float mx = -INFINITY;
+  for (int c = tid; c < P.vocab; c += MTT) mx = fmaxf(mx, x[c]);
+  mx = block_reduce_max(sm, mx);
+  float su = 0.f;
+  for (int c = tid; c < P.vocab; c += MTT) su += expf(x[c] - mx);
+  su = block_reduce_sum(sm, su);
+  const float lse = logf(su);
+  float best = -INFINITY;
+  int bi = 0x7fffffff;
+  for (int c = tid; c < P.vocab; c += MTT) {
+    const bool masked = (c == P.pad) || (s < 1 && c == P.eos);
+    float lp = masked ? -INFINITY : (x[c] - mx) - lse;
+    if (lp > best || (lp == best && c < bi)) {
+      best = lp;
+      bi = c;
+    }
+  }
+#pragma unroll
+  for (int o = 16; o > 0; o >>= 1) {
+    float ob = __shfl_xor_sync(0xffffffffu, best, o);
+    int oi = __shfl_xor_sync(0xffffffffu, bi, o);
+    if (ob > best || (ob == best && oi < bi)) {
+      best = ob;
+      bi = oi;
+    }
+  }
+  __syncthreads();
+  if ((tid & 31) == 0) {
+    sm.rbest[tid >> 5] = best;
+    sm.ridx[tid >> 5] = bi;
+  }
+  __syncthreads();
+  if (tid == 0) {
+    for (int i = 1; i < MW; ++i)
+      if (sm.rbest[i] > best || (sm.rbest[i] == best && sm.ridx[i] < bi)) {
+        best = sm.rbest[i];
+        bi = sm.ridx[i];
+      }
+    sm.tok = bi;
+    if (blockIdx.x == 0) P.tok[s + 1] = bi;
+  }
+  __syncthreads();
 }
 
 __global__ void __launch_bounds__(MTT, 1) mt_decode_persistent_kernel(MtDecodeParams P, const MtLayerP* __restrict__ layers, int step0,
@@ -310,49 +356,7 @@
     BAR();
     if (forced_eos) break;
     {
-      const float* x = P.logits;
-      float mx = -INFINITY;
-      for (int c = tid; c < P.vocab; c += MTT) mx = fmaxf(mx, x[c]);
-      mx = block_reduce_max(sm, mx);
-      float su = 0.f;
-      for (int c = tid; c < P.vocab; c += MTT) su += expf(x[c] - mx);
-      su = block_reduce_sum(sm, su);
-      const float lse = logf(su);
-      float best = -INFINITY;
-      int bi = 0x7fffffff;
-      for (int c = tid; c < P.vocab; c += MTT) {
-        const bool masked = (c == P.pad) || (s < 1 && c == P.eos);
-        float lp = masked ? -INFINITY : (x[c] - mx) - lse;
-        if (lp > best || (lp == best && c < bi)) {
-          best = lp;
-          bi = c;
-        }
-      }
-#pragma unroll
-      for (int o = 16; o > 0; o >>= 1) {
-        float ob = __shfl_xor_sync(0xffffffffu, best, o);
-        int oi = __shfl_xor_sync(0xffffffffu, bi, o);
-        if (ob > best || (ob == best && oi < bi)) {
-          best = ob;
-          bi = oi;
-        }
-      }
-      __syncthreads();
-      if ((tid & 31) == 0) {
-        sm.rbest[tid >> 5] = best;
-        sm.ridx[tid >> 5] = bi;
-      }
-      __syncthreads();
-      if (tid == 0) {
-        for (int i = 1; i < MW; ++i)
-          if (sm.rbest[i] > best || (sm.rbest[i] == best && sm.ridx[i] < bi)) {
-            best = sm.rbest[i];
-            bi = sm.ridx[i];
-          }
-        sm.tok = bi;
-        if (blockIdx.x == 0) P.tok[s + 1] = bi;
-      }
-      __syncthreads();
+      greedy_argmax(sm, P, s, P.logits);
       if (sm.tok == P.eos) break;
     }
   }
@@ -365,13 +369,15 @@
 constexpr int PCOLS = 512 / GRP;
 constexpr int PCOLS_PER_WARP = PCOLS / MW;
 
-__device__ void attend_head_early(MtSmem& sm, const float* q, const float* kbase, const float* vbase, int ld, int n, float* out) {
+template <bool PART = false>
+__device__ void attend_head_early(MtSmem& sm, const float* q, const float* kbase, const float* vbase, int ld, int n, float* out,
+                                  const float* klast = nullptr, const float* vlast = nullptr) {
   const int tid = threadIdx.x;
   const int q4 = (tid & 15) * 4, part = tid >> 4;
   float4 kk[MHD / 4];
   {
     const bool ok = tid < n;
-    const float* kr = kbase + (int64_t)(ok ? tid : 0) * ld;
+    const float* kr = (PART && klast && tid == n - 1) ? klast : kbase + (int64_t)(ok ? tid : 0) * ld;
 #pragma unroll
     for (int d = 0; d < MHD / 4; ++d) kk[d] = ok ? *reinterpret_cast<const float4*>(kr + 4 * d) : make_float4(0.f, 0.f, 0.f, 0.f);
   }
@@ -379,7 +385,8 @@
 #pragma unroll
   for (int u = 0; u < 8; ++u) {
     const int j = part + 16 * u;
-    vv0[u] = j < n ? *reinterpret_cast<const float4*>(vbase + (int64_t)j * ld + q4) : make_float4(0.f, 0.f, 0.f, 0.f);
+    const float* vr = (PART && klast && j == n - 1) ? vlast : vbase + (int64_t)j * ld;
+    vv0[u] = j < n ? *reinterpret_cast<const float4*>(vr + q4) : make_float4(0.f, 0.f, 0.f, 0.f);
   }
   __syncthreads();
   if (tid < MHD) sm.qh[tid] = q[tid] * 0.125f;
@@ -387,7 +394,7 @@
   float mx = -INFINITY;
   for (int j = tid; j < n; j += MTT) {
     if (j != tid) {
-      const float* kr = kbase + (int64_t)j * ld;
+      const float* kr = (PART && klast && j == n - 1) ? klast : kbase + (int64_t)j * ld;
 #pragma unroll
       for (int d = 0; d < MHD / 4; ++d) kk[d] = *reinterpret_cast<const float4*>(kr + 4 * d);
     }
@@ -419,7 +426,8 @@
     for (int u = 0; u < 8; ++u) {
       const int j = j0 + 16 * u;
       const bool ok = j < n;
-      vv[u] = j0 == part ? vv0[u] : (ok ? *reinterpret_cast<const float4*>(vbase + (int64_t)j * ld + q4) : make_float4(0.f, 0.f, 0.f, 0.f));
+      const float* vr = (PART && klast && j == n - 1) ? vlast : vbase + (int64_t)j * ld;
+      vv[u] = j0 == part ? vv0[u] : (ok ? *reinterpret_cast<const float4*>(vr + q4) : make_float4(0.f, 0.f, 0.f, 0.f));
       pp[u] = ok ? sm.S[j] : 0.f;
     }
 #pragma unroll
@@ -436,45 +444,63 @@
     float t = 0.f;
 #pragma unroll
     for (int x = 0; x < 16; ++x) t += sm.pv[x][tid];
-    out[tid] = t / sum;
-  }
-}
-
+    out[tid] = PART ? t : t / sum;
+  }
+  if (PART && tid == 0) {
+    out[MHD] = mx;
+    out[MHD + 1] = sum;
+  }
+}
+
+template <int NC = PCOLS_PER_WARP>
 struct HpW {
-  float w0[PCOLS_PER_WARP], w1[PCOLS_PER_WARP];
+  float w0[NC], w1[NC];
 };
 
-__device__ __forceinline__ HpW hp_load(const float* __restrict__ W, int h, int j) {
+template <int NC = PCOLS_PER_WARP>
+__device__ __forceinline__ HpW<NC> hp_load(const float* __restrict__ W, int h, int j) {
   const int lane = threadIdx.x & 31, warp = threadIdx.x >> 5;
-  HpW r;
-#pragma unroll
-  for (int c = 0; c < PCOLS_PER_WARP; ++c) {
-    const float* w = W + (int64_t)(j * PCOLS + warp * PCOLS_PER_WARP + c) * 512 + h * MHD;
+  HpW<NC> r;
+#pragma unroll
+  for (int c = 0; c < NC; ++c) {
+    const float* w = W + (int64_t)(j * NC * MW + warp * NC + c) * 512 + h * MHD;
     r.w0[c] = __ldg(w + lane);
     r.w1[c] = __ldg(w + lane + 32);
   }
   return r;
 }
-__device__ __forceinline__ void head_partial_proj_w(const float* a, const HpW& hw, int j, float* part_h) {
+template <int NC>
+__device__ __forceinline__ void head_partial_proj_w(const float* a, const HpW<NC>& hw, int j, float* part_h) {
   const int lane = threadIdx.x & 31, warp = threadIdx.x >> 5;
   const float a0 = a[lane], a1 = a[lane + 32];
 #pragma unroll
-  for (int c = 0; c < PCOLS_PER_WARP; ++c) {
+  for (int c = 0; c < NC; ++c) {
     float acc = fmaf(a0, hw.w0[c], a1 * hw.w1[c]);
     acc = warp_sum(acc);
-    if (lane == 0) part_h[j * PCOLS + warp * PCOLS_PER_WARP + c] = acc;
+    if (lane == 0) part_h[j * NC * MW + warp * NC + c] = acc;
   }
 }
 
 __device__ __forceinline__ void add_head_partials(MtSmem& sm, const float* part, const float* __restrict__ bias) {
-  for (int c = threadIdx.x; c < 512; c += MTT) {
-    float t = part[c];
-#pragma unroll
-    for (int h = 1; h < 8; ++h) t += part[h * 512 + c];
-    sm.x[c] = sm.x[c] + (t + (bias ? bias[c] : 0.f));
-  }
-  __syncthreads();
-}
+  float p[2][8], b[2];
+#pragma unroll
+  for (int i = 0; i < 2; ++i) {
+    const int c = threadIdx.x + i * MTT;
+#pragma unroll
+    for (int h = 0; h < 8; ++h) p[i][h] = part[h * 512 + c];
+    b[i] = bias ? __ldg(bias + c) : 0.f;
+  }
+#pragma unroll
+  for (int i = 0; i < 2; ++i) {
+    const int c = threadIdx.x + i * MTT;
+    float t = p[i][0];
+#pragma unroll
+    for (int h = 1; h < 8; ++h) t += p[i][h];
+    sm.x[c] = sm.x[c] + (t + b[i]);
+  }
+  __syncthreads();
+}
+static_assert(2 * MTT == 512, "add_head_partials: two columns per thread");
 
 template <int K, int MAXC>
 __device__ __forceinline__ void gemv_prefetch(const float* __restrict__ W, int N) {
@@ -593,7 +619,7 @@
       });
       STAMP(1);
       ARRIVE();
-      HpW hw;
+      HpW<> hw;
       if (in_group) hw = hp_load(L.wo, grp_h, grp_j);
       WAIT();
       STAMP(2);
@@ -665,49 +691,7 @@
     BAR();
     if (forced_eos) break;
     {
-      const float* x = P.logits;
-      float mx = -INFINITY;
-      for (int c = tid; c < P.vocab; c += MTT) mx = fmaxf(mx, x[c]);
-      mx = block_reduce_max(sm, mx);
-      float su = 0.f;
-      for (int c = tid; c < P.vocab; c += MTT) su += expf(x[c] - mx);
-      su = block_reduce_sum(sm, su);
-      const float lse = logf(su);
-      float best = -INFINITY;
-      int bi = 0x7fffffff;
-      for (int c = tid; c < P.vocab; c += MTT) {
-        const bool masked = (c == P.pad) || (s < 1 && c == P.eos);
-        float lp = masked ? -INFINITY : (x[c] - mx) - lse;
-        if (lp > best || (lp == best && c < bi)) {
-          best = lp;
-          bi = c;
-        }
-      }
-#pragma unroll
-      for (int o = 16; o > 0; o >>= 1) {
-        float ob = __shfl_xor_sync(0xffffffffu, best, o);
-        int oi = __shfl_xor_sync(0xffffffffu, bi, o);
-        if (ob > best || (ob == best && oi < bi)) {
-          best = ob;
-          bi = oi;
-        }
-      }
-      __syncthreads();
-      if ((tid & 31) == 0) {
-        sm.rbest[tid >> 5] = best;
-        sm.ridx[tid >> 5] = bi;
-      }
-      __syncthreads();
-      if (tid == 0) {
-        for (int i = 1; i < MW; ++i)
-          if (sm.rbest[i] > best || (sm.rbest[i] == best && sm.ridx[i] < bi)) {
-            best = sm.rbest[i];
-            bi = sm.ridx[i];
-          }
-        sm.tok = bi;
-        if (blockIdx.x == 0) P.tok[s + 1] = bi;
-      }
-      __syncthreads();
+      greedy_argmax(sm, P, s, P.logits);
       if (sm.tok == P.eos) break;
     }
   }
@@ -719,6 +703,387 @@
   if (threadIdx.x == 0 && done_barriers < planned) atomicAdd(bar_ctr, (unsigned)(planned - done_barriers));
 }
 
+constexpr int CL_CS = 8;
+constexpr int CL_GRID = 8 * CL_CS;
+constexpr int CL_QKV = 3 * MHD / CL_CS;
+constexpr int CL_CQ = MHD / CL_CS;
+constexpr int CL_PC = 512 / CL_CS;
+constexpr int CL_HID = 2048 / CL_GRID;
+constexpr int CL_W2LD = CL_HID + 4;
+constexpr int CL_OUT = 96;
+constexpr int CL_OUTW = CL_OUT / MW;
+enum { XC_QKV = 0, XC_CQ = 1, XC_FFN = 2, XC_ATT = 3, XC_N = 4 };
+
+struct MtClSmem {
+  MtSmem m;
+  alignas(16) float qkv[3 * MHD];
+  alignas(16) float cq[MHD];
+  alignas(16) float red[CL_CS][CL_PC];
+  alignas(16) float att[MHD];
+  float attl[MHD + 2];
+  float attp[CL_CS][MHD + 2];
+  alignas(16) float hid[CL_HID];
+  unsigned long long xbar[XC_N];
+  alignas(16) float wbuf[CL_OUT * 512];
+};
+static_assert(CL_HID * 512 + 512 * CL_W2LD <= CL_OUT * 512, "FFN staging");
+static_assert(offsetof(MtClSmem, qkv) % 16 == 0 && offsetof(MtClSmem, hid) % 16 == 0 && offsetof(MtClSmem, wbuf) % 16 == 0, "float4 access");
+
+__device__ __forceinline__ void cp_async16(void* smem, const void* g) {
+  asm volatile("cp.async.cg.shared.global [%0], [%1], 16;" ::"r"(smem_u32(smem)), "l"(g) : "memory");
+}
+__device__ __forceinline__ void cp_async_wait_all() { asm volatile("cp.async.wait_all;" ::: "memory"); }
+
+template <int MAXC>
+struct ClRows {
+  float4 w[MAXC][4];
+  float b[MAXC];
+};
+template <int MAXC, int N, typename R>
+__device__ __forceinline__ void cl_issue(ClRows<MAXC>& r, const float* __restrict__ W, const float* __restrict__ bias, R&& row) {
+  const int lane = threadIdx.x & 31, warp = threadIdx.x >> 5;
+#pragma unroll
+  for (int c = 0; c < MAXC; ++c) {
+    const int k = warp + MW * c;
+    if (k < N) {
+      const int64_t rr = row(k);
+#pragma unroll
+      for (int it = 0; it < 4; ++it) r.w[c][it] = ldw(W + rr * 512 + it * 128 + lane * 4);
+      r.b[c] = bias ? __ldg(bias + rr) : 0.f;
+    }
+  }
+}
+template <int MAXC, int N, typename F>
+__device__ __forceinline__ void cl_finish(const ClRows<MAXC>& r, const float* xs, F&& epi) {
+  const int lane = threadIdx.x & 31, warp = threadIdx.x >> 5;
+  float4 xv[4];
+#pragma unroll
+  for (int it = 0; it < 4; ++it) xv[it] = *reinterpret_cast<const float4*>(xs + it * 128 + lane * 4);
+#pragma unroll
+  for (int c = 0; c < MAXC; ++c) {
+    const int k = warp + MW * c;
+    if (k < N) {
+      float acc = 0.f;
+#pragma unroll
+      for (int it = 0; it < 4; ++it) {
+        acc = fmaf(xv[it].x, r.w[c][it].x, acc);
+        acc = fmaf(xv[it].y, r.w[c][it].y, acc);
+        acc = fmaf(xv[it].z, r.w[c][it].z, acc);
+        acc = fmaf(xv[it].w, r.w[c][it].w, acc);
+      }
+      epi(k, warp_sum(acc) + r.b[c]);
+    }
+  }
+}
+template <int MAXC, typename F>
+__device__ __forceinline__ void cl_smem_rows(const float* Ws, const float* xs, int n, F&& epi) {
+  const int lane = threadIdx.x & 31, warp = threadIdx.x >> 5;
+  float4 xv[4];
+#pragma unroll
+  for (int it = 0; it < 4; ++it) xv[it] = *reinterpret_cast<const float4*>(xs + it * 128 + lane * 4);
+#pragma unroll 4
+  for (int c = 0; c < MAXC; ++c) {
+    const int k = warp + MW * c;
+    if (k < n) {
+      float acc = 0.f;
+#pragma unroll
+      for (int it = 0; it < 4; ++it) {
+        const float4 w = *reinterpret_cast<const float4*>(Ws + k * 512 + it * 128 + lane * 4);
+        acc = fmaf(xv[it].x, w.x, acc);
+        acc = fmaf(xv[it].y, w.y, acc);
+        acc = fmaf(xv[it].z, w.z, acc);
+        acc = fmaf(xv[it].w, w.w, acc);
+      }
+      epi(k, warp_sum(acc));
+    }
+  }
+}
+
+template <typename R>
+__device__ __forceinline__ void cl_prefetch(int n, int lines, R&& row) {
+  for (int i = threadIdx.x; i < n * lines; i += MTT) asm volatile("prefetch.global.L2 [%0];" ::"l"(row(i / lines) + (i % lines) * 32));
+}
+
+__device__ __forceinline__ int cl_qkv_row(int h, int i) { return (i >> 6) * 512 + h * MHD + (i & 63); }
+
+__device__ __forceinline__ void cl_layer_prefetch(const MtLayerP& L, int h, int r) {
+  const int u0 = (h * CL_CS + r) * CL_HID;
+  cl_prefetch(CL_QKV, 16, [&](int k) { return L.wqkv + (int64_t)cl_qkv_row(h, r * CL_QKV + k) * 512; });
+  cl_prefetch(CL_CQ, 16, [&](int k) { return L.wcq + (int64_t)(h * MHD + r * CL_CQ + k) * 512; });
+  cl_prefetch(CL_PC, 2, [&](int k) { return L.wo + (int64_t)(r * CL_PC + k) * 512 + h * MHD; });
+  cl_prefetch(CL_PC, 2, [&](int k) { return L.wco + (int64_t)(r * CL_PC + k) * 512 + h * MHD; });
+  cl_prefetch(CL_HID, 16, [&](int k) { return L.w1 + (int64_t)(u0 + k) * 512; });
+  cl_prefetch(512, 1, [&](int k) { return L.w2 + (int64_t)k * 2048 + u0; });
+}
+
+__device__ __forceinline__ void cl_stage_ffn(MtClSmem& sm, const MtLayerP& L, int u0) {
+  for (int i = threadIdx.x; i < CL_HID * 128; i += MTT) cp_async16(sm.wbuf + i * 4, L.w1 + (int64_t)u0 * 512 + i * 4);
+  float* w2s = sm.wbuf + CL_HID * 512;
+  for (int i = threadIdx.x; i < 512 * (CL_HID / 4); i += MTT) {
+    const int o = i / (CL_HID / 4), q = i % (CL_HID / 4);
+    cp_async16(w2s + o * CL_W2LD + q * 4, L.w2 + (int64_t)o * 2048 + u0 + q * 4);
+  }
+}
+
+__global__ void __launch_bounds__(MTT, 1) mt_decode_cluster_kernel(MtDecodeParams P, const MtLayerP* __restrict__ layers, int step0, int nsteps,
+                                                                   int max_len, int T, unsigned* bar_ctr, unsigned bar_target) {
+  extern __shared__ __align__(128) unsigned char dyn[];
+  MtClSmem& cs = *reinterpret_cast<MtClSmem*>(dyn);
+  MtSmem& sm = cs.m;
+  constexpr int DIM = 512;
+  const int tid = threadIdx.x, lane = tid & 31;
+  const int barriers_per_step = P.n_layers * 3 + 1;
+  int done_barriers = 0;
+  const float emb_scale = sqrtf((float)DIM);
+  const int h = blockIdx.x / CL_CS, r = blockIdx.x % CL_CS;
+  const int u0 = blockIdx.x * CL_HID;
+  float* part_attn = P.part_cl;
+  float* part_cross = P.part_cl + 8 * DIM;
+  float* part_ffn = P.part_cl + 16 * DIM;
+  if (tid == 0) {
+    for (int i = 0; i < XC_N; ++i) asm volatile("mbarrier.init.shared::cta.b64 [%0], 1;" ::"r"(smem_u32(&cs.xbar[i])));
+    asm volatile("fence.mbarrier_init.release.cluster;" ::: "memory");
+  }
+  cluster_sync();
+  unsigned xph = 0;
+
+  auto xwait = [&](int ch, uint32_t bytes) {
+    const uint32_t bar = smem_u32(&cs.xbar[ch]);
+    if (tid == 0) asm volatile("mbarrier.arrive.expect_tx.shared::cta.b64 _, [%0], %1;" ::"r"(bar), "r"(bytes) : "memory");
+    mbar_wait(bar, (xph >> ch) & 1u);
+    xph ^= 1u << ch;
+  };
+  auto attend = [&](const float* q, const float* kb, const float* vb, int ld, int n, bool self) {
+    const int chunk = (n + CL_CS - 1) / CL_CS;
+    const int j0 = min(n, r * chunk), cnt = min(n, j0 + chunk) - j0;
+    const bool last = self && cnt > 0 && j0 + cnt == n;
+    attend_head_early<true>(sm, q, kb + (int64_t)j0 * ld, vb + (int64_t)j0 * ld, ld, cnt, cs.attl, last ? cs.qkv + MHD : nullptr,
+                            last ? cs.qkv + 2 * MHD : nullptr);
+    __syncthreads();
+    if (tid < MHD + 2)
+      for (int k = 0; k < CL_CS; ++k) st_peer(&cs.attp[r][tid], k, cs.attl[tid], &cs.xbar[XC_ATT]);
+    xwait(XC_ATT, CL_CS * (MHD + 2) * 4);
+    if (tid < MHD) {
+      float m = cs.attp[0][MHD];
+#pragma unroll
+      for (int i = 1; i < CL_CS; ++i) m = fmaxf(m, cs.attp[i][MHD]);
+      float o = 0.f, l = 0.f;
+#pragma unroll
+      for (int i = 0; i < CL_CS; ++i) {
+        const float e = expf(cs.attp[i][MHD] - m);
+        o = fmaf(cs.attp[i][tid], e, o);
+        l = fmaf(cs.attp[i][MHD + 1], e, l);
+      }
+      cs.att[tid] = o / l;
+    }
+    __syncthreads();
+  };
+#define BAR()                          \
+  grid_barrier(bar_ctr, bar_target);   \
+  ++done_barriers;
+#define ARRIVE()                       \
+  grid_arrive(bar_ctr, bar_target);    \
+  ++done_barriers;
+#define WAIT() grid_wait(bar_ctr, bar_target)
+  int nts = 0;
+  bool stamping = false;
+#define STAMP(id)                                          \
+  if (stamping && tid == 0) {                              \
+    unsigned long long t_;                                 \
+    asm volatile("mov.u64 %0, %%globaltimer;" : "=l"(t_)); \
+    P.ts[1 + 2 * nts] = (id);                              \
+    P.ts[2 + 2 * nts] = t_;                                \
+    ++nts;                                                 \
+    P.ts[0] = nts;                                         \
+  }
+  ClRows<3> w_qkv;
+  HpW<CL_PC / MW> w_o;
+  LnP ln_self;
+  auto issue_self = [&](const MtLayerP& Ln) {
+    cl_issue<3, CL_QKV>(w_qkv, Ln.wqkv, Ln.bqkv, [&](int k) { return cl_qkv_row(h, r * CL_QKV + k); });
+    w_o = hp_load<CL_PC / MW>(Ln.wo, h, r);
+    ln_self = ln_load(Ln.self_g, Ln.self_b);
+  };
+  issue_self(layers[0]);
+  const int out_row0 = blockIdx.x * CL_OUT, out_rows = max(0, min(CL_OUT, P.vocab - out_row0));
+  for (int si = 0; si < nsteps; ++si) {
+    const int s = step0 + si;
+    {
+      const int64_t tok = (si == 0) ? P.tok[s] : (int64_t)sm.tok;
+      const int p = (tok == P.pad) ? P.pad : P.pad + 1 + s;
+      for (int c = tid; c < DIM; c += MTT) sm.x[c] = emb_scale * P.emb[tok * DIM + c] + P.pos[(int64_t)p * DIM + c];
+      __syncthreads();
+    }
+    for (int l = 0; l < P.n_layers; ++l) {
+      const MtLayerP L = layers[l];
+      stamping = P.ts != nullptr && blockIdx.x == 0 && si == 1 && l == 1;
+      STAMP(20);
+      if (l + 1 < P.n_layers) cl_layer_prefetch(layers[l + 1], h, r);
+      else {
+        cl_prefetch(CL_OUT, 16, [&](int k) { return P.emb + (int64_t)min(blockIdx.x * CL_OUT + k, P.vocab - 1) * DIM; });
+        if (si + 1 < nsteps) cl_layer_prefetch(layers[0], h, r);
+      }
+      if (l > 0) add_head_partials(sm, part_ffn, layers[l - 1].b2);
+      ln_to_v(sm, ln_self, DIM);
+      {
+        float* kc = P.self_k + ((size_t)l * P.max_pos + s + P.kv_off) * DIM + h * MHD;
+        float* vc = P.self_v + ((size_t)l * P.max_pos + s + P.kv_off) * DIM + h * MHD;
+        cl_finish<3, CL_QKV>(w_qkv, sm.v, [&](int k, float y) {
+          const int i = r * CL_QKV + k;
+          if (lane < CL_CS) st_peer(&cs.qkv[i], lane, y, &cs.xbar[XC_QKV]);
+          if (lane == 0 && i >= MHD) {
+            if (i < 2 * MHD) kc[i - MHD] = y;
+            else vc[i - 2 * MHD] = y;
+          }
+        });
+      }
+      STAMP(21);
+      xwait(XC_QKV, 3 * MHD * 4);
+      attend(cs.qkv, P.self_k + (size_t)l * P.max_pos * DIM + h * MHD, P.self_v + (size_t)l * P.max_pos * DIM + h * MHD, DIM, s + P.kv_off + 1,
+             true);
+      head_partial_proj_w(cs.att, w_o, r, part_attn + h * DIM);
+      STAMP(22);
+      ARRIVE();
+      ClRows<1> w_cq;
+      cl_issue<1, CL_CQ>(w_cq, L.wcq, L.bcq, [&](int k) { return h * MHD + r * CL_CQ + k; });
+      const LnP ln_cross = ln_load(L.cross_g, L.cross_b);
+      HpW<CL_PC / MW> w_co = hp_load<CL_PC / MW>(L.wco, h, r);
+      cl_stage_ffn(cs, L, u0);
+      WAIT();
+      STAMP(23);
+      add_head_partials(sm, part_attn, L.bo);
+      ln_to_v(sm, ln_cross, DIM);
+      cl_finish<1, CL_CQ>(w_cq, sm.v, [&](int k, float y) {
+        if (lane < CL_CS) st_peer(&cs.cq[r * CL_CQ + k], lane, y, &cs.xbar[XC_CQ]);
+      });
+      xwait(XC_CQ, MHD * 4);
+      {
+        const float* cross = P.cross_kv + (size_t)l * P.cross_cap * 2 * DIM;
+        attend(cs.cq, cross + h * MHD, cross + DIM + h * MHD, 2 * DIM, T, false);
+      }
+      head_partial_proj_w(cs.att, w_co, r, part_cross + h * DIM);
+      STAMP(24);
+      ARRIVE();
+      const LnP ln_fin = ln_load(L.fin_g, L.fin_b);
+      const float b1v = L.b1 ? __ldg(L.b1 + u0 + lane) : 0.f;
+      WAIT();
+      STAMP(25);
+      add_head_partials(sm, part_cross, L.bco);
+      ln_to_v(sm, ln_fin, DIM);
+      cp_async_wait_all();
+      __syncthreads();
+      cl_smem_rows<CL_HID / MW>(cs.wbuf, sm.v, CL_HID, [&](int k, float acc) {
+        const float y = acc + __shfl_sync(0xffffffffu, b1v, k);
+        if (lane == 0) cs.hid[k] = y > 0.f ? y : 0.f;
+      });
+      __syncthreads();
+      {
+        const float* w2s = cs.wbuf + CL_HID * 512;
+        float4 hv[CL_HID / 4];
+#pragma unroll
+        for (int q = 0; q < CL_HID / 4; ++q) hv[q] = *reinterpret_cast<const float4*>(&cs.hid[4 * q]);
+#pragma unroll
+        for (int half = 0; half < 2; ++half) {
+          const int o = tid + half * MTT;
+          float acc = 0.f;
+#pragma unroll
+          for (int q = 0; q < CL_HID / 4; ++q) {
+            const float4 w = *reinterpret_cast<const float4*>(w2s + o * CL_W2LD + 4 * q);
+            acc = fmaf(hv[q].x, w.x, acc);
+            acc = fmaf(hv[q].y, w.y, acc);
+            acc = fmaf(hv[q].z, w.z, acc);
+            acc = fmaf(hv[q].w, w.w, acc);
+          }
+          st_peer(&cs.red[r][o % CL_PC], o / CL_PC, acc, &cs.xbar[XC_FFN]);
+        }
+      }
+      __syncthreads();
+      const bool last = l + 1 == P.n_layers;
+      if (last && s < max_len)
+        for (int i = tid; i < out_rows * 128; i += MTT) cp_async16(cs.wbuf + i * 4, P.emb + (int64_t)out_row0 * DIM + i * 4);
+      xwait(XC_FFN, CL_CS * CL_PC * 4);
+      if (tid < CL_PC) {
+        float t = cs.red[0][tid];
+#pragma unroll
+        for (int src = 1; src < CL_CS; ++src) t += cs.red[src][tid];
+        part_ffn[h * DIM + r * CL_PC + tid] = t;
+      }
+      STAMP(26);
+      ARRIVE();
+      if (!last) issue_self(layers[l + 1]);
+      WAIT();
+      STAMP(27);
+    }
+    const bool forced_eos = s >= max_len;
+    const LnP ln_out = ln_load(P.out_g, P.out_b);
+    add_head_partials(sm, part_ffn, layers[P.n_layers - 1].b2);
+    ln_to_v(sm, ln_out, DIM);
+    if (blockIdx.x == 0)
+      for (int c = tid; c < DIM; c += MTT) P.feats[(size_t)s * DIM + c] = sm.v[c];
+    if (!forced_eos) {
+      cp_async_wait_all();
+      __syncthreads();
+      cl_smem_rows<CL_OUTW>(cs.wbuf, sm.v, out_rows, [&](int k, float acc) {
+        if (lane == 0) P.logits[out_row0 + k] = acc;
+      });
+    }
+    ARRIVE();
+    if (!forced_eos && si + 1 < nsteps) issue_self(layers[0]);
+    WAIT();
+    if (forced_eos) break;
+    for (int c = tid; c < P.vocab; c += MTT) cs.wbuf[c] = P.logits[c];
+    __syncthreads();
+    greedy_argmax(sm, P, s, cs.wbuf);
+    if (sm.tok == P.eos) break;
+  }
+#undef BAR
+#undef ARRIVE
+#undef WAIT
+#undef STAMP
+  cp_async_wait_all();
+  const int planned = nsteps * barriers_per_step;
+  if (threadIdx.x == 0 && done_barriers < planned) atomicAdd(bar_ctr, (unsigned)(planned - done_barriers));
+  cluster_sync();
+}
+
+bool mt_decode_cluster_launch(const MtDecodeParams& P, const MtLayerP* layers_dev, int step0, int nsteps, int max_len, int T, unsigned* bar_ctr,
+                              unsigned* bar_target_host, cudaStream_t st) {
+  static int fits[64] = {0};
+  int dev = 0;
+  cudaGetDevice(&dev);
+  if (dev < 0 || dev >= 64 || P.vocab > CL_GRID * CL_OUT) return false;
+  const size_t smem = sizeof(MtClSmem);
+  cudaLaunchConfig_t cfg{};
+  cfg.gridDim = dim3(CL_GRID);
+  cfg.blockDim = dim3(MTT);
+  cfg.dynamicSmemBytes = smem;
+  cfg.stream = st;
+  cudaLaunchAttribute attr[2];
+  attr[0].id = cudaLaunchAttributeClusterDimension;
+  attr[0].val.clusterDim.x = CL_CS;
+  attr[0].val.clusterDim.y = 1;
+  attr[0].val.clusterDim.z = 1;
+  attr[1].id = cudaLaunchAttributeCooperative;
+  attr[1].val.cooperative = 1;
+  cfg.attrs = attr;
+  cfg.numAttrs = 2;
+  if (fits[dev] == 0) {
+    int max_clusters = 0;
+    const bool ok = cudaFuncSetAttribute(mt_decode_cluster_kernel, cudaFuncAttributeMaxDynamicSharedMemorySize, (int)smem) == cudaSuccess &&
+                    cudaOccupancyMaxActiveClusters(&max_clusters, mt_decode_cluster_kernel, &cfg) == cudaSuccess && max_clusters >= 8;
+    cudaGetLastError();
+    fits[dev] = ok ? 1 : -1;
+  }
+  if (fits[dev] < 0) return false;
+  MtDecodeParams p = P;
+  if (cudaLaunchKernelEx(&cfg, mt_decode_cluster_kernel, p, layers_dev, step0, nsteps, max_len, T, bar_ctr, *bar_target_host) != cudaSuccess) {
+    cudaGetLastError();
+    return false;
+  }
+  *bar_target_host += (unsigned)CL_GRID * (unsigned)(nsteps * (P.n_layers * 3 + 1));
+  return true;
+}
+
 }
 
 bool mt_decode_persistent_supported(int dim, int ffn, int heads, int vocab, int max_pos, int T) {
@@ -728,6 +1093,7 @@
 int mt_decode_persistent(const MtDecodeParams& P, const MtLayerP* layers_dev, int step0, int nsteps, int max_len, int T, unsigned* bar_ctr,
                          unsigned* bar_target_host, cudaStream_t st) {
   ++g_launches;
+  if (P.part_cl != nullptr && P.heads == 8 && mt_decode_cluster_launch(P, layers_dev, step0, nsteps, max_len, T, bar_ctr, bar_target_host, st)) return 0;
   int occ = 0;
   if (first_time_on_device((const void*)mt_decode_persistent_kernel)) {
     cudaOccupancyMaxActiveBlocksPerMultiprocessor(&occ, mt_decode_persistent_kernel, MTT, 0);
diff --git a/streamspeech_b200/engine.py b/streamspeech_b200/engine.py
--- a/streamspeech_b200/engine.py
+++ b/streamspeech_b200/engine.py
@@ -190,6 +190,7 @@
         self.set_option("persistent_encoder_cluster", int(os.environ.get("SS_PERSISTENT_ENCODER_CLUSTER", "1")))
         self.set_option("cluster_cooperative", int(os.environ.get("SS_CLUSTER_COOPERATIVE", "1")))
         self.set_option("persistent_mt_v2", int(os.environ.get("SS_PERSISTENT_MT_V2", "1")))
+        self.set_option("persistent_mt_cluster", int(os.environ.get("SS_PERSISTENT_MT_CLUSTER", "1")))
         self.set_option("persistent_mt_prefix", int(os.environ.get("SS_PERSISTENT_MT_PREFIX", "1")))
         self.set_option("vocoder_streams", int(os.environ.get("SS_VOCODER_STREAMS", "1")))
         self.set_option("unit_grouped", int(os.environ.get("SS_UNIT_GROUPED", "1")))
```

New measurement: 136.6, median of 6. 1.03x the previous value.
